# JunweiLiang/Multiverse

Measured on AMD Instinct MI355X. Metric: trajectories/sec (8-obs/12-pred, multi-scale 18x32+9x16 grid, greedy forward), higher is better.
Workload: dtype f16x3 (fp32 operands as two pre-scaled fp16 planes, fp32 accumulate and state; winograd F(3,3) over image rows on pre-transformed operands, 1.67 fp16 MFMAs issued per fp32 product over the gate kernels; error vs fp64 within 2x of the fp32-MFMA path's -- asserted under checkpoint-like dynamic range (; 1 GPU; BASELINE configs[1]: multi-scale 18x32+9x16 (scene 36x64x11), batch 64/GPU, fp32 forward-only, beam 1, obs 8 / pred 12; gate convolution on the fp16 matrix pipe (f16x3 split, fp32-class error); batch_per_gpu=64, global_batch=64, obs_len=8, pred_len=12, parallelism=batch-sharded x1, no data-path collective

## Files before the change

### multiverse_amd/csrc/engine.hip

```cpp
#include "../../include/multiverse_hip.h"

#include <hip/hip_runtime.h>

#include <cmath>
#include <cstdio>
#include <cstdlib>
#include <cstring>
#include <algorithm>
#include <map>
#include <memory>
#include <mutex>
#include <set>
#include <string>
#include <tuple>
#include <vector>

#include "convlstm_mfma.h"
#include "convlstm_wgrad.h"
#include "convlstm_f16x3.h"
#include "convlstm_wino.h"
#include "convlstm_wino3.h"
#include "convlstm_generic.h"
#include "convlstm_wgrad_f16x3.h"
#include "kernels_misc.h"
#include "decode_tail.h"
#include "sparse_x.h"
#include "multifuture_decode.h"
#include "train_kernels.h"
#include "comm.h"

#include "engine_state.h"
#include "gate_plan.h"
#include "engine_setup.h"
#include "engine_forward.h"
#include "engine_io.h"


#include "engine_train.h"

namespace {

struct OpCtx {
  int device;
  hipStream_t stream = nullptr;
  explicit OpCtx(int dev) : device(dev) {
    HIP_CHECK(hipSetDevice(dev));
    HIP_CHECK(hipStreamCreate(&stream));
  }
  ~OpCtx() { if (stream) (void)hipStreamDestroy(stream); }
  template <typename T>
  void up(DevBuf<T>& b, const T* src, size_t n) {
    b.alloc(n ? n : 1);
    if (n) HIP_CHECK(hipMemcpy(b.p, src, n * sizeof(T), hipMemcpyHostToDevice));
  }
  template <typename T>
  void down(T* dst, const DevBuf<T>& b, size_t n) {
    HIP_CHECK(hipStreamSynchronize(stream));
    if (n) HIP_CHECK(hipMemcpy(dst, b.p, n * sizeof(T), hipMemcpyDeviceToHost));
  }
};

}


extern "C" {

int mv_abi_version(void) { return MV_ABI_VERSION; }

const char* mv_last_error(mv_handle h) {
  return h ? h->err.c_str() : g_create_error.c_str();
}

int mv_create(const mv_config* cfg, int device, mv_handle* out) {
  if (!cfg || !out) { g_create_error = "mv_create: NULL argument"; return 1; }
  *out = nullptr;
  mv_engine* e = nullptr;
  int rc = guarded(nullptr, [&] {
    validate_config(*cfg);
    int ndev = 0;
    HIP_CHECK(hipGetDeviceCount(&ndev));
    MV_REQUIRE(device >= 0 && device < ndev, "device %d not in [0,%d)", device, ndev);
    HIP_CHECK(hipSetDevice(device));
    hipDeviceProp_t prop;
    HIP_CHECK(hipGetDeviceProperties(&prop, device));
    MV_REQUIRE(strncmp(prop.gcnArchName, "gfx950", 6) == 0,
               "device %d is %s; this library contains gfx950 (MI355X) code only",
               device, prop.gcnArchName);
    e = new mv_engine();
    e->cfg = *cfg;
    e->device = device;
    HIP_CHECK(hipStreamCreate(&e->stream));
    build_param_table(e);
    alloc_buffers(e);
    if (cfg->beam_size > 1) {
      size_t K = 0;
      for (int s = 0; s < cfg->num_scales; ++s)
        if (e->sc[s].use) K = e->sc[s].K;
      ensure_beam_step_lds(device, ((size_t)2 * cfg->beam_size * K + 512) * sizeof(float));
    }
  });
  if (rc != 0) { delete e; return rc; }
  *out = e;
  return 0;
}

int mv_destroy(mv_handle h) {
  if (!h) return 0;
  (void)hipSetDevice(h->device);
  if (h->stream) (void)hipStreamSynchronize(h->stream);
  if (h->copy_stream) (void)hipStreamSynchronize(h->copy_stream);
  if (h->fetch_stream) (void)hipStreamSynchronize(h->fetch_stream);
  pipeline_destroy(h);
  h->drop_graphs();
  if (h->comm) {
    if (h->comm->stream) (void)hipStreamSynchronize(h->comm->stream);
    if (h->comm->comm) (void)mv::rccl().CommDestroy(h->comm->comm);
    if (h->comm->ready) (void)hipEventDestroy(h->comm->ready);
    if (h->comm->done) (void)hipEventDestroy(h->comm->done);
    if (h->comm->stream) (void)hipStreamDestroy(h->comm->stream);
    delete h->comm;
  }
  delete h->train;
  if (h->stream) (void)hipStreamDestroy(h->stream);
  delete h;
  return 0;
}

int mv_num_params(mv_handle h) { return h ? (int)h->params.size() : -1; }

int mv_param_info(mv_handle h, int32_t i, char* name_out, int32_t name_cap,
                  int64_t* shape_out) {
  if (!h || i < 0 || i >= (int)h->params.size()) return -1;
  Param* p = h->params[i].get();
  if (name_out && name_cap > 0) {
    strncpy(name_out, p->name.c_str(), name_cap - 1);
    name_out[name_cap - 1] = 0;
  }
  if (shape_out)
    for (size_t d = 0; d < 4; ++d) shape_out[d] = d < p->shape.size() ? p->shape[d] : 0;
  return (int)p->shape.size();
}

int mv_set_param(mv_handle h, const char* tf_name, const float* data,
                 const int64_t* shape, int32_t rank) {
  if (!h) return 1;
  return guarded(h, [&] {
    MV_REQUIRE(tf_name && data && shape, "mv_set_param: NULL argument");
    auto it = h->by_name.find(tf_name);
    MV_REQUIRE(it != h->by_name.end(), "unknown parameter '%s'", tf_name);
    Param* p = it->second;
    MV_REQUIRE(rank == (int)p->shape.size(), "parameter %s: rank %d, expected %zu",
               tf_name, rank, p->shape.size());
    for (int d = 0; d < rank; ++d)
      MV_REQUIRE(shape[d] == p->shape[d], "parameter %s: dim %d is %lld, expected %lld",
                 tf_name, d, (long long)shape[d], (long long)p->shape[d]);
    const size_t n = p->elems();
    p->host.assign(data, data + n);
    p->dev.alloc(n);
    HIP_CHECK(hipMemcpy(p->dev.p, data, n * sizeof(float), hipMemcpyHostToDevice));
    p->set = true;
    h->drop_graphs();
    h->train_packs_valid = false;
    for (int s = 0; s < h->cfg.num_scales; ++s) h->sc[s].wq_valid = h->sc[s].sx_valid = false;
    for (int s = 0; s < h->cfg.num_scales; ++s) {
      ScaleState& S = h->sc[s];
      for (ConvCell* cc : {&S.enc_cls, &S.enc_reg, &S.dec_cls, &S.dec_reg})
        if (cc->kernel == p) {
          cc->wpack.release(); cc->wp16.release(); cc->wx32.release();
          cc->wpb.release(); cc->wpbt.release(); cc->wx32u.release(); cc->wpw.release(); cc->wpw3.release();
          cc->host_stale = false;
        }
    }
  });
}

int mv_get_param(mv_handle h, const char* tf_name, float* out, int64_t capacity) {
  if (!h) return 1;
  return guarded(h, [&] {
    MV_REQUIRE(tf_name && out, "mv_get_param: NULL argument");
    auto it = h->by_name.find(tf_name);
    MV_REQUIRE(it != h->by_name.end(), "unknown parameter '%s'", tf_name);
    Param* p = it->second;
    MV_REQUIRE(p->set, "parameter %s not set", tf_name);
    MV_REQUIRE((size_t)capacity >= p->elems(), "buffer too small for %s", tf_name);
    HIP_CHECK(hipMemcpy(out, p->dev.p, p->elems() * sizeof(float), hipMemcpyDeviceToHost));
  });
}

int mv_upload_inputs(mv_handle h, const mv_inputs* in) {
  if (!h) return 1;
  return guarded(h, [&] {
    MV_REQUIRE(in, "mv_upload_inputs: NULL inputs");
    upload_inputs(h, in);
  });
}

int mv_set_grid_centers(mv_handle h, int32_t scale, const double* centers) {
  if (!h) return 1;
  return guarded(h, [&] {
    MV_REQUIRE(scale >= 0 && scale < h->cfg.num_scales && h->sc[scale].use,
               "mv_set_grid_centers: scale %d is not an enabled scale", scale);
    MV_REQUIRE(centers, "mv_set_grid_centers: NULL centers");
    ScaleState& S = h->sc[scale];
    S.centers.alloc((size_t)S.K * 2);
    HIP_CHECK(hipMemcpy(S.centers.p, centers, (size_t)S.K * 2 * sizeof(double),
                        hipMemcpyHostToDevice));
  });
}

int mv_upload_inputs_compact(mv_handle h, const mv_inputs_compact* in) {
  if (!h) return 1;
  return guarded(h, [&] {
    MV_REQUIRE(in, "mv_upload_inputs_compact: NULL inputs");
    upload_inputs_compact(h, in);
  });
}

int mv_run_greedy_resident(mv_handle h) {
  if (!h) return 1;
  return guarded(h, [&] {
    MV_REQUIRE(h->cfg.beam_size == 1, "engine was created for beam search");
    run_forward(h, false);
  });
}

int mv_run_beam_resident(mv_handle h) {
  if (!h) return 1;
  return guarded(h, [&] { run_forward(h, true); });
}

int mv_synchronize(mv_handle h) {
  if (!h) return 1;
  return guarded(h, [&] {
    HIP_CHECK(hipStreamSynchronize(h->stream));
    drain_events(h);
  });
}

int mv_download_outputs(mv_handle h, mv_outputs* out) {
  if (!h) return 1;
  return guarded(h, [&] {
    MV_REQUIRE(out, "NULL outputs");
    download_outputs(h, out);
  });
}

int mv_download_beam_outputs(mv_handle h, mv_beam_outputs* out) {
  if (!h) return 1;
  return guarded(h, [&] {
    MV_REQUIRE(out, "NULL outputs");
    download_beam(h, out);
  });
}

int mv_decode_trajectories(mv_handle h, int32_t scale, int32_t center_only, double* out) {
  if (!h) return 1;
  return guarded(h, [&] {
    decode_trajectories(h, scale, center_only != 0, out);
    drain_events(h);
  });
}

int mv_beam_occupancy(mv_handle h, float* out) {
  if (!h) return 1;
  return guarded(h, [&] {
    beam_occupancy(h, out);
    drain_events(h);
  });
}

int mv_download_beam_ids(mv_handle h, int32_t* ids, float* logprobs) {
  if (!h) return 1;
  return guarded(h, [&] {
    download_beam_ids(h, ids, logprobs);
    drain_events(h);
  });
}

int mv_forward_greedy(mv_handle h, const mv_inputs* in, mv_outputs* out) {
  if (!h) return 1;
  return guarded(h, [&] {
    MV_REQUIRE(in && out, "mv_forward_greedy: NULL argument");
    MV_REQUIRE(h->cfg.beam_size == 1, "engine was created for beam search");
    upload_inputs(h, in);
    run_forward(h, false);
    download_outputs(h, out);
    drain_events(h);
  });
}

int mv_pipeline_create(mv_handle h, int32_t depth) {
  if (!h) return 1;
  return guarded(h, [&] { pipeline_create(h, depth); });
}

int mv_submit_greedy(mv_handle h, const mv_inputs* in) {
  if (!h) return 1;
  return guarded(h, [&] {
    MV_REQUIRE(in, "mv_submit_greedy: NULL argument");
    pipeline_submit(h, in);
  });
}

int mv_collect_greedy(mv_handle h, mv_outputs* out, int32_t* pred_len) {
  if (!h) return 1;
  return guarded(h, [&] {
    MV_REQUIRE(out, "mv_collect_greedy: NULL argument");
    if (pred_len && !h->pipe.empty())
      *pred_len = h->pipe[h->pipe_tail % h->pipe.size()].pred_len;
    pipeline_collect(h, out);
    drain_events(h);
  });
}

int mv_forward_beam(mv_handle h, const mv_inputs* in, mv_beam_outputs* out) {
  if (!h) return 1;
  return guarded(h, [&] {
    MV_REQUIRE(in && out, "mv_forward_beam: NULL argument");
    upload_inputs(h, in);
    run_forward(h, true);
    download_beam(h, out);
    drain_events(h);
  });
}

int mv_set_profiling(mv_handle h, int32_t enabled) {
  if (!h) return 1;
  h->profiling = enabled != 0;
  return 0;
}

int mv_train_init(mv_handle h, const mv_train_config* tc) {
  if (!h) return 1;
  return guarded(h, [&] {
    MV_REQUIRE(tc, "mv_train_init: NULL config");
    MV_REQUIRE(tc->optimizer >= 0 && tc->optimizer <= 3, "Optimizer not implemented: %d "
               "(0 adadelta, 1 momentum, 2 adam, 3 rmsprop; reference pred_models.py:1667-1681)",
               tc->optimizer);
    MV_REQUIRE(tc->class_feedback >= 0 && tc->class_feedback <= 2, "class_feedback %d",
               tc->class_feedback);
    MV_REQUIRE(tc->keep_prob > 0.f && tc->keep_prob <= 1.f, "keep_prob %g not in (0, 1]",
               tc->keep_prob);
    if (tc->use_soft_grid_class)
      MV_REQUIRE(tc->soft_kernel_size == 3 || tc->soft_kernel_size == 5,
                 "soft_kernel_size %d (3 or 5)", tc->soft_kernel_size);
    MV_REQUIRE(h->cfg.beam_size == 1, "training needs a greedy (beam_size 1) engine "
               "(reference pred_models.py:261)");
    if (!h->train) {
      h->train = new mv_train_holder();
      train_alloc(h);
      h->drop_graphs();
      for (int s = 0; s < h->cfg.num_scales; ++s) h->sc[s].wq_valid = h->sc[s].sx_valid = false;
    }
    TrainState& t = h->train->st;
    t.tc = *tc;
    if (t.slots_for != tc->optimizer) {
      HIP_CHECK(hipMemsetAsync(t.accum.p, 0, t.total_elems * sizeof(float), h->stream));
      HIP_CHECK(hipMemsetAsync(t.accum_update.p, 0, t.total_elems * sizeof(float), h->stream));
      if (tc->optimizer == 3)
        hipLaunchKernelGGL(mv::fill_kernel, dim3(cdiv(t.total_elems, 256)), dim3(256), 0,
                           h->stream, t.accum.p, 1.0f, t.total_elems);
      t.beta1_power = 0.9f; t.beta2_power = 0.999f;
      HIP_CHECK(hipStreamSynchronize(h->stream));
      t.slots_for = tc->optimizer;
    }
  });
}

int mv_train_forward_backward(mv_handle h, const mv_inputs* in, const mv_targets* tg,
                              mv_losses* out) {
  if (!h) return 1;
  return guarded(h, [&] {
    MV_REQUIRE((in == nullptr) == (tg == nullptr),
               "mv_train_forward_backward: give both inputs and targets, or neither "
               "(resident)");
    train_fwd_bwd(h, in, tg, out);
  });
}

int mv_upload_targets(mv_handle h, const mv_targets* tg) {
  if (!h) return 1;
  return guarded(h, [&] {
    MV_REQUIRE(h->train, "mv_train_init has not been called");
    MV_REQUIRE(tg, "mv_upload_targets: NULL targets");
    MV_REQUIRE(h->inputs_ready, "mv_upload_inputs first (it fixes T_pred)");
    upload_targets(h, tg);
    TS(h).targets_ready = true;
  });
}

int mv_upload_targets_compact(mv_handle h, const mv_targets_compact* tg) {
  if (!h) return 1;
  return guarded(h, [&] {
    MV_REQUIRE(h->train, "mv_train_init has not been called");
    MV_REQUIRE(tg, "mv_upload_targets_compact: NULL targets");
    MV_REQUIRE(h->inputs_ready, "mv_upload_inputs first (it fixes T_pred)");
    upload_targets_compact(h, tg);
    TS(h).targets_ready = true;
  });
}

int mv_train_apply(mv_handle h, float grad_scale) {
  if (!h) return 1;
  return guarded(h, [&] { train_apply(h, grad_scale); });
}

int mv_train_step(mv_handle h, const mv_inputs* in, const mv_targets* tg, mv_losses* out) {
  if (!h) return 1;
  return guarded(h, [&] {
    MV_REQUIRE((in == nullptr) == (tg == nullptr),
               "mv_train_step: give both inputs and targets, or neither (resident)");
    train_fwd_bwd(h, in, tg, out);
    train_apply(h, h->comm ? 1.0f / (float)h->comm->world : 1.0f);
  });
}

int mv_grad_buffer(mv_handle h, float** device_ptr, int64_t* elems) {
  if (!h) return 1;
  return guarded(h, [&] {
    MV_REQUIRE(h->train, "mv_train_init has not been called");
    MV_REQUIRE(device_ptr && elems, "mv_grad_buffer: NULL argument");
    *device_ptr = TS(h).grad.p;
    *elems = (int64_t)TS(h).total_elems;
  });
}

static Param* find_param(mv_handle h, const char* tf_name) {
  MV_REQUIRE(tf_name, "NULL parameter name");
  auto it = h->by_name.find(tf_name);
  MV_REQUIRE(it != h->by_name.end(), "unknown parameter '%s'", tf_name);
  return it->second;
}

int mv_get_grad(mv_handle h, const char* tf_name, float* out, int64_t capacity) {
  if (!h) return 1;
  return guarded(h, [&] {
    MV_REQUIRE(h->train && TS(h).have_grads, "no gradients (mv_train_forward_backward)");
    Param* p = find_param(h, tf_name);
    MV_REQUIRE(out && (size_t)capacity >= p->elems(), "buffer too small for %s", tf_name);
    HIP_CHECK(hipMemcpy(out, grad_of(h, p), p->elems() * sizeof(float),
                        hipMemcpyDeviceToHost));
  });
}

int mv_get_global_step(mv_handle h, int64_t* step) {
  if (!h || !step || !h->train) return 1;
  *step = h->train->st.global_step;
  return 0;
}

int mv_set_global_step(mv_handle h, int64_t step) {
  if (!h || !h->train) return 1;
  h->train->st.global_step = step;
  return 0;
}

int mv_comm_unique_id(uint8_t* id_out) {
  return guarded(nullptr, [&] {
    MV_REQUIRE(id_out, "mv_comm_unique_id: NULL buffer");
    mv::RcclApi& r = mv::rccl();
    MV_REQUIRE(r.ok, "RCCL unavailable: %s", r.error.c_str());
    ncclUniqueId id;
    ncclResult_t rc = r.GetUniqueId(&id);
    MV_REQUIRE(rc == ncclSuccess, "ncclGetUniqueId: %s", r.GetErrorString(rc));
    static_assert(sizeof(id) == MV_COMM_ID_BYTES, "ncclUniqueId size");
    memcpy(id_out, &id, sizeof(id));
  });
}

int mv_allreduce_init(mv_handle h, int32_t rank, int32_t world, const uint8_t* unique_id) {
  if (!h) return 1;
  return guarded(h, [&] {
    MV_REQUIRE(unique_id && world >= 1 && rank >= 0 && rank < world,
               "mv_allreduce_init: bad arguments (rank %d of %d)", rank, world);
    MV_REQUIRE(!h->comm, "mv_allreduce_init: communicator already initialised");
    mv::RcclApi& r = mv::rccl();
    MV_REQUIRE(r.ok, "RCCL unavailable: %s", r.error.c_str());
    std::unique_ptr<mv::Comm> c(new mv::Comm());
    c->rank = rank; c->world = world;
    ncclUniqueId id;
    memcpy(&id, unique_id, sizeof(id));
    ncclResult_t rc = r.CommInitRank(&c->comm, world, id, rank);
    MV_REQUIRE(rc == ncclSuccess, "ncclCommInitRank(rank %d of %d): %s", rank, world,
               r.GetErrorString(rc));
    HIP_CHECK(hipStreamCreateWithFlags(&c->stream, hipStreamNonBlocking));
    HIP_CHECK(hipEventCreateWithFlags(&c->ready, hipEventDisableTiming));
    HIP_CHECK(hipEventCreateWithFlags(&c->done, hipEventDisableTiming));
    h->comm = c.release();
  });
}

int mv_allreduce_info(mv_handle h, int32_t* rank, int32_t* world, int32_t* buckets,
                      double* bytes) {
  if (!h || !h->comm) return 1;
  if (rank) *rank = h->comm->rank;
  if (world) *world = h->comm->world;
  if (buckets) *buckets = h->comm->buckets_last;
  if (bytes) *bytes = h->comm->bytes_last;
  return 0;
}

int mv_attack_begin(mv_handle h) {
  if (!h) return 1;
  return guarded(h, [&] {
    MV_REQUIRE(!h->no_scene(), "mv_attack_begin: the model has no scene encoder (scene_conv_dim 0): "
               "there are no scene features");
    MV_REQUIRE(h->train, "mv_train_init has not been called");
    MV_REQUIRE(h->inputs_ready, "no inputs uploaded");
    TrainState& t = TS(h);
    const size_t n = (size_t)h->num_frames * h->cfg.scene_h * h->cfg.scene_w * h->cfg.scene_class;
    t.scene_clean.alloc((size_t)h->cfg.batch_size * h->cfg.obs_len * h->cfg.scene_h *
                        h->cfg.scene_w * h->cfg.scene_class);
    HIP_CHECK(hipMemcpyAsync(t.scene_clean.p, h->scene_feat.p, n * sizeof(float),
                             hipMemcpyDeviceToDevice, h->stream));
    t.want_dscene = true;
    t.have_dscene = false;
  });
}

int mv_attack_end(mv_handle h) {
  if (!h || !h->train) return 1;
  TS(h).want_dscene = false;
  return 0;
}

int mv_set_scene_feat(mv_handle h, const float* scene_feat) {
  if (!h) return 1;
  return guarded(h, [&] {
    MV_REQUIRE(!h->no_scene(), "mv_set_scene_feat: the model has no scene encoder (scene_conv_dim 0): "
               "there are no scene features");
    MV_REQUIRE(scene_feat && h->inputs_ready, "mv_set_scene_feat: NULL / no inputs uploaded");
    const size_t n = (size_t)h->num_frames * h->cfg.scene_h * h->cfg.scene_w * h->cfg.scene_class;
    HIP_CHECK(hipMemcpy(h->scene_feat.p, scene_feat, n * sizeof(float), hipMemcpyHostToDevice));
  });
}

int mv_get_scene_feat(mv_handle h, float* out) {
  if (!h) return 1;
  return guarded(h, [&] {
    MV_REQUIRE(!h->no_scene(), "mv_get_scene_feat: the model has no scene encoder (scene_conv_dim 0): "
               "there are no scene features");
    MV_REQUIRE(out && h->inputs_ready, "mv_get_scene_feat: NULL / no inputs uploaded");
    const size_t n = (size_t)h->num_frames * h->cfg.scene_h * h->cfg.scene_w * h->cfg.scene_class;
    HIP_CHECK(hipStreamSynchronize(h->stream));
    HIP_CHECK(hipMemcpy(out, h->scene_feat.p, n * sizeof(float), hipMemcpyDeviceToHost));
  });
}

int mv_get_scene_grad(mv_handle h, float* out) {
  if (!h) return 1;
  return guarded(h, [&] {
    MV_REQUIRE(!h->no_scene(), "mv_get_scene_grad: the model has no scene encoder (scene_conv_dim 0): "
               "there are no scene features");
    MV_REQUIRE(h->train && TS(h).have_dscene, "no input gradient (mv_attack_begin, then "
               "mv_train_forward_backward)");
    const size_t n = (size_t)h->num_frames * h->cfg.scene_h * h->cfg.scene_w * h->cfg.scene_class;
    HIP_CHECK(hipStreamSynchronize(h->stream));
    HIP_CHECK(hipMemcpy(out, TS(h).dscene.p, n * sizeof(float), hipMemcpyDeviceToHost));
  });
}

int mv_attack_step(mv_handle h, float epsilon, float step) {
  if (!h) return 1;
  return guarded(h, [&] {
    MV_REQUIRE(!h->no_scene(), "mv_attack_step: the model has no scene encoder (scene_conv_dim 0): "
               "there are no scene features");
    MV_REQUIRE(h->train && TS(h).have_dscene && TS(h).scene_clean.p,
               "mv_attack_step: mv_attack_begin + mv_train_forward_backward first");
    const size_t n = (size_t)h->num_frames * h->cfg.scene_h * h->cfg.scene_w * h->cfg.scene_class;
    hipLaunchKernelGGL(mv::adv_step_kernel, dim3(cdiv(n, 256)), dim3(256), 0, h->stream,
                       h->scene_feat.p, TS(h).dscene.p, TS(h).scene_clean.p, epsilon, step, n);
    HIP_CHECK(hipGetLastError());
  });
}

int mv_scene_mix(mv_handle h, const float* other, float weight) {
  if (!h) return 1;
  return guarded(h, [&] {
    MV_REQUIRE(!h->no_scene(), "mv_scene_mix: the model has no scene encoder (scene_conv_dim 0): "
               "there are no scene features");
    MV_REQUIRE(h->train && h->inputs_ready, "mv_scene_mix: training engine with inputs");
    const size_t n = (size_t)h->num_frames * h->cfg.scene_h * h->cfg.scene_w * h->cfg.scene_class;
    TrainState& t = TS(h);
    const float* src = t.scene_clean.p;
    DevBuf<float> tmp;
    if (other) {
      tmp.alloc(n);
      HIP_CHECK(hipMemcpy(tmp.p, other, n * sizeof(float), hipMemcpyHostToDevice));
      src = tmp.p;
    }
    MV_REQUIRE(src, "mv_scene_mix: no clean copy (mv_attack_begin)");
    hipLaunchKernelGGL(mv::mix_kernel, dim3(cdiv(n, 256)), dim3(256), 0, h->stream,
                       h->scene_feat.p, src, weight, n);
    HIP_CHECK(hipStreamSynchronize(h->stream));
  });
}

int mv_get_sample_losses(mv_handle h, int32_t scale, float* out) {
  if (!h) return 1;
  return guarded(h, [&] {
    MV_REQUIRE(h->train && TS(h).have_grads, "no losses (mv_train_forward_backward)");
    MV_REQUIRE(scale >= 0 && scale < h->cfg.num_scales && h->sc[scale].use && out,
               "mv_get_sample_losses: scale %d", scale);
    const int N = h->cfg.batch_size, Tp = h->pred_len;
    TrainState& t = TS(h);
    hipLaunchKernelGGL(mv::loss_rows_mean_kernel, dim3(cdiv(N, 256)), dim3(256), 0, h->stream,
                       t.sc[scale].loss_row.p, t.scratch.p, Tp, N);
    HIP_CHECK(hipStreamSynchronize(h->stream));
    HIP_CHECK(hipMemcpy(out, t.scratch.p, N * sizeof(float), hipMemcpyDeviceToHost));
  });
}

int mv_set_label_mixup(mv_handle h, const int32_t* const* obs_labels2,
                       const int32_t* const* pred_labels2, float weight,
                       const float* sample_weight) {
  if (!h) return 1;
  return guarded(h, [&] {
    MV_REQUIRE(!h->no_scene(), "mv_set_label_mixup: not built for a model without the scene encoder "
               "(scene_conv_dim 0)");
    MV_REQUIRE(h->train, "mv_train_init has not been called");
    MV_REQUIRE(obs_labels2 && pred_labels2, "mv_set_label_mixup: NULL argument");
    MV_REQUIRE(weight >= 0.f && weight <= 1.f, "mv_set_label_mixup: weight %g not in [0, 1]",
               (double)weight);
    TrainState& t = TS(h);
    const int N = h->cfg.batch_size, To = h->cfg.obs_len, Tp = h->pred_len;
    for (int s = 0; s < h->cfg.num_scales; ++s) {
      if (!h->sc[s].use) continue;
      MV_REQUIRE(obs_labels2[s] && pred_labels2[s], "mv_set_label_mixup: scale %d is NULL", s);
      const int K = h->sc[s].K;
      for (int i = 0; i < N * To; ++i)
        MV_REQUIRE(obs_labels2[s][i] >= 0 && obs_labels2[s][i] < K,
                   "mv_set_label_mixup: observed label %d out of range", obs_labels2[s][i]);
      for (int i = 0; i < N * Tp; ++i)
        MV_REQUIRE(pred_labels2[s][i] >= 0 && pred_labels2[s][i] < K,
                   "mv_set_label_mixup: future label %d out of range", pred_labels2[s][i]);
      HIP_CHECK(hipMemcpy(t.sc[s].obs_labels2.p, obs_labels2[s], (size_t)N * To * sizeof(int32_t),
                          hipMemcpyHostToDevice));
      HIP_CHECK(hipMemcpy(t.sc[s].pred_labels2.p, pred_labels2[s],
                          (size_t)N * Tp * sizeof(int32_t), hipMemcpyHostToDevice));
    }
    if (sample_weight)
      HIP_CHECK(hipMemcpy(t.sample_w.p, sample_weight, (size_t)N * sizeof(float),
                          hipMemcpyHostToDevice));
    t.mix_on = true; t.mix_sw = sample_weight != nullptr; t.mix_w = weight;
  });
}

int mv_clear_label_mixup(mv_handle h) {
  if (!h || !h->train) return 1;
  TS(h).mix_on = TS(h).mix_sw = false;
  TS(h).mix_w = 1.f;
  return 0;
}

int mv_set_dropout_seed(mv_handle h, uint32_t seed) {
  if (!h || !h->train) return 1;
  h->train->st.dropout_seed = seed;
  return 0;
}

int mv_get_opt_scalars(mv_handle h, float* beta1_power, float* beta2_power) {
  if (!h || !h->train || !beta1_power || !beta2_power) return 1;
  *beta1_power = h->train->st.beta1_power;
  *beta2_power = h->train->st.beta2_power;
  return 0;
}

int mv_set_opt_scalars(mv_handle h, float beta1_power, float beta2_power) {
  if (!h || !h->train) return 1;
  h->train->st.beta1_power = beta1_power;
  h->train->st.beta2_power = beta2_power;
  return 0;
}

int mv_get_opt_slot(mv_handle h, const char* tf_name, int32_t slot, float* out,
                    int64_t capacity) {
  if (!h) return 1;
  return guarded(h, [&] {
    MV_REQUIRE(h->train, "mv_train_init has not been called");
    MV_REQUIRE(slot == 0 || slot == 1, "slot must be 0 or 1 (see multiverse_hip.h)");
    Param* p = find_param(h, tf_name);
    MV_REQUIRE(out && (size_t)capacity >= p->elems(), "buffer too small for %s", tf_name);
    const float* src = (slot == 0 ? TS(h).accum.p : TS(h).accum_update.p) +
                       TS(h).goff[param_index(h, p)];
    HIP_CHECK(hipMemcpy(out, src, p->elems() * sizeof(float), hipMemcpyDeviceToHost));
  });
}

int mv_set_opt_slot(mv_handle h, const char* tf_name, int32_t slot, const float* data,
                    int64_t elems) {
  if (!h) return 1;
  return guarded(h, [&] {
    MV_REQUIRE(h->train, "mv_train_init has not been called");
    MV_REQUIRE(slot == 0 || slot == 1, "slot must be 0 or 1 (see multiverse_hip.h)");
    Param* p = find_param(h, tf_name);
    MV_REQUIRE(data && (size_t)elems == p->elems(), "size mismatch for %s", tf_name);
    float* dst = (slot == 0 ? TS(h).accum.p : TS(h).accum_update.p) +
                 TS(h).goff[param_index(h, p)];
    HIP_CHECK(hipMemcpy(dst, data, p->elems() * sizeof(float), hipMemcpyHostToDevice));
  });
}

int mv_set_compute_mode(mv_handle h, int32_t mode) {
  if (!h) return 1;
  return guarded(h, [&] {
    MV_REQUIRE(mode >= 0 && mode <= 2, "compute mode %d (0 = fp32 MFMA, 1 = f16x3, 2 = bf16)",
               mode);
    MV_REQUIRE(mode == 0 || h->cfg.convlstm_kernel == 3,
               "compute mode %d needs convlstm_kernel 3 (%d given: the matrix-pipe gate kernels "
               "are 3 x 3 stencils; mode 0 runs the generic fp32 loops)", mode,
               h->cfg.convlstm_kernel);
    if (mode != 0) {
      const mv_config& c = h->cfg;
      size_t K = 0;
      for (int s = 0; s < c.num_scales; ++s)
        if (h->sc[s].use) K = std::max(K, (size_t)h->sc[s].K);
      const size_t xc = (size_t)std::max(c.scene_conv_dim, c.emb_size);
      for (int i = 0; i < mv::kMaxGroup; ++i) {
        const size_t rows = (size_t)c.batch_size * ((i % 2 == 0) ? c.beam_size : 1);
        h->px16[i].alloc(2 * (rows * K * xc + mv::kPlaneSlack + mv::kPlanePad));
        h->ph16[i].alloc(2 * (rows * K * c.hidden_size + mv::kPlaneSlack + mv::kPlanePad));
        HIP_CHECK(hipMemset(h->px16[i].p, 0, h->px16[i].n * sizeof(_Float16)));
        if (c.activation != 0) h->xexp[i].alloc(65);
        if (wino3_possible(mode, c.activation)) {
          size_t vx = 0, vh = 0;
          for (int s = 0; s < c.num_scales; ++s) {
            if (!h->sc[s].use) continue;
            vx = std::max(vx, wino3_scratch_elems((int)rows, h->sc[s].H, h->sc[s].W, (int)xc));
            vh = std::max(vh, wino3_scratch_elems((int)rows, h->sc[s].H, h->sc[s].W, c.hidden_size));
          }
          if (vx) h->pv3x[i].alloc(vx);
          if (vh) h->pv3h[i].alloc(vh);
        }
        HIP_CHECK(hipMemset(h->ph16[i].p, 0, h->ph16[i].n * sizeof(_Float16)));
      }
    }
    if (mode != 0 && h->planes.empty()) {
      for (int s = 0; s < h->cfg.num_scales; ++s) {
        ScaleState& S = h->sc[s];
        if (!S.use) continue;
        for (DevBuf<float>* b : {&S.cls_h[0], &S.cls_h[1], &S.reg_h[0], &S.reg_h[1],
                                 &S.cls_hg, &S.xbuf_cls, &S.xbuf_reg}) {
          if (!b->p) continue;
          h->plane_store.emplace_back(new DevBuf<_Float16>());
          DevBuf<_Float16>& pb = *h->plane_store.back();
          pb.alloc(2 * (b->n + mv::kPlaneSlack + mv::kPlanePad));
          HIP_CHECK(hipMemset(pb.p, 0, pb.n * sizeof(_Float16)));
          h->planes[b->p] = mv_engine::PlaneBuf{pb.p + mv::kPlanePad,
                                                b->n + mv::kPlaneSlack + mv::kPlanePad, false};
          if (b == &S.xbuf_cls || b == &S.xbuf_reg) h->xbufs.insert(b->p);
        }
      }
    }
    for (auto& kv : h->planes) kv.second.valid = false;
    if (h->compute_mode != mode) {
      h->drop_graphs();
      h->train_packs_valid = false;
    }
    h->compute_mode = mode;
  });
}

int mv_set_graph_mode(mv_handle h, int32_t enabled) {
  if (!h) return 1;
  h->graph_mode = enabled != 0;
  return 0;
}

int mv_reset_kernel_stats(mv_handle h) {
  if (!h) return 1;
  return guarded(h, [&] {
    HIP_CHECK(hipStreamSynchronize(h->stream));
    drain_events(h);
    h->stats.clear();
  });
}

int mv_num_kernel_stats(mv_handle h) { return h ? (int)h->stats.size() : -1; }

int mv_kernel_stat_dense_flops(mv_handle h, int32_t i, double* flops_dense) {
  if (!h || i < 0 || i >= (int)h->stats.size() || !flops_dense) return 1;
  *flops_dense = h->stats[i].flops_dense;
  return 0;
}

int mv_kernel_stat_mfma_flops(mv_handle h, int32_t i, double* flops_mfma) {
  if (!h || i < 0 || i >= (int)h->stats.size() || !flops_mfma) return 1;
  *flops_mfma = h->stats[i].flops_mfma;
  return 0;
}

int mv_kernel_stat(mv_handle h, int32_t i, char* name_out, int32_t name_cap,
                   int64_t* launches, double* total_ms, double* flops, double* bytes) {
  if (!h || i < 0 || i >= (int)h->stats.size()) return 1;
  const KernelStat& s = h->stats[i];
  if (name_out && name_cap > 0) {
    strncpy(name_out, s.name.c_str(), name_cap - 1);
    name_out[name_cap - 1] = 0;
  }
  if (launches) *launches = s.launches;
  if (total_ms) *total_ms = s.total_ms;
  if (flops) *flops = s.flops;
  if (bytes) *bytes = s.bytes;
  return 0;
}

static int time_resident(mv_handle h, int32_t iters, float* ms_out, bool beam) {
  if (!h) return 1;
  return guarded(h, [&] {
    MV_REQUIRE(iters >= 1 && ms_out, "bad arguments");
    hipEvent_t a, b;
    HIP_CHECK(hipEventCreate(&a));
    HIP_CHECK(hipEventCreate(&b));
    HIP_CHECK(hipEventRecord(a, h->stream));
    for (int i = 0; i < iters; ++i) run_forward(h, beam);
    HIP_CHECK(hipEventRecord(b, h->stream));
    HIP_CHECK(hipEventSynchronize(b));
    HIP_CHECK(hipEventElapsedTime(ms_out, a, b));
    (void)hipEventDestroy(a);
    (void)hipEventDestroy(b);
    drain_events(h);
  });
}

int mv_time_greedy_resident(mv_handle h, int32_t iters, float* ms_out) {
  return time_resident(h, iters, ms_out, false);
}
int mv_time_beam_resident(mv_handle h, int32_t iters, float* ms_out) {
  return time_resident(h, iters, ms_out, true);
}

}

#include "engine_ops.h"
```

### multiverse_amd/csrc/engine_forward.h

```cpp
#pragma once

namespace {


using mv::ConvLstmArgs;

void set_sparse_x(mv_engine* e, ScaleState& S, ConvLstmArgs& a, bool decoder,
                  const int32_t* hot, int hot_stride, int hot_div) {
  a.sx_bias = decoder ? S.sx_dec_bias.p : nullptr;
  a.sx_corr = decoder ? S.sx_dec_corr.p : S.sx_enc_corr.p;
  a.sx_hot = hot; a.sx_hot_stride = hot_stride; a.sx_hot_div = hot_div;
  a.sx_cellyx = S.sx_cellyx.p;
  a.sx_rad = decoder ? 2 : 1;
  a.sx_by_class = decoder ? 1 : 0;
}

ConvLstmArgs conv_problem(mv_engine* e, const ConvCell& cc, const float* x,
                          const float* h, const float* c, const int32_t* src_row_h,
                          const int32_t* src_row_c, float* h_out, float* c_out,
                          int rows, int H, int W, bool zero_state,
                          size_t x_row_stride = 0, bool want_h16 = true) {
  ConvLstmArgs a{};
  const size_t xrs = x_row_stride ? x_row_stride : (size_t)H * W * cc.Cx;
  MV_REQUIRE((size_t)rows * H * W * e->cfg.hidden_size < ((size_t)1 << 31) &&
             (size_t)rows * xrs < ((size_t)1 << 31),
             "ConvLSTM state of %d rows exceeds the 2^31-element addressing of one "
             "launch; lower batch_size x beam_size", rows);
  a.x_row_stride = (int32_t)xrs;
  a.x = x; a.h = h; a.c = c; a.src_row_h = src_row_h; a.src_row_c = src_row_c;
  a.wpack = cc.wpack.p; a.bias = cc.biases->dev.p;
  a.h_out = h_out; a.c_out = c_out;
  a.rows = rows; a.H = H; a.W = W; a.Cx = cc.Cx; a.C = e->cfg.hidden_size;
  mv::convlstm_finish_args(a, zero_state);
  a.want_h16 = want_h16 ? 1 : 0;
  return a;
}

ConvCell* cell_of_bias(mv_engine* e, const float* bias) {
  for (int s = 0; s < e->cfg.num_scales; ++s) {
    ScaleState& S = e->sc[s];
    if (!S.use) continue;
    for (ConvCell* cc : active_cells(e, S))
      if (cc->biases && cc->biases->dev.p == bias) return cc;
  }
  throw HipError{"internal: unknown ConvLSTM cell"};
}

ConvCell* cell_of_pack(mv_engine* e, const float* wpack) {
  for (int s = 0; s < e->cfg.num_scales; ++s) {
    ScaleState& S = e->sc[s];
    for (ConvCell* cc : active_cells(e, S))
      if (cc->wpack.p == wpack) return cc;
  }
  throw HipError{"internal: unknown weight pack"};
}


void prepare_gate_operands(mv_engine* e, const std::vector<ConvLstmArgs>& probs,
                           const std::vector<ConvCell*>& cells,
                           std::vector<mv::ConvLstm16Args>& p16) {
  struct SplitItem { const float* in; _Float16* p0; _Float16* p1; int cells, C; };
  std::vector<SplitItem> splits;
  struct DynItem { const float* in; _Float16* p0; _Float16* p1; int cells, C; int32_t* bits; };
  std::vector<DynItem> dyn_splits;
  const bool bf16 = e->compute_mode == 2;
  auto ready = [&](const float* src) -> const mv_engine::PlaneBuf* {
    auto it = e->planes.find(src);
    return (it != e->planes.end() && it->second.valid) ? &it->second : nullptr;
  };
  for (size_t i = 0; i < probs.size(); ++i) {
    const ConvLstmArgs& a = probs[i];
    mv::ConvLstm16Args& q = p16[i];
    MV_REQUIRE(a.H * a.W >= 32, "f16x3 / bf16 compute modes need grids of at least 32 cells "
               "(%d x %d); use compute mode f32", a.H, a.W);
    MV_REQUIRE((double)a.rows * a.H * a.W * a.C * 4.0 < 4294967296.0,
               "f16x3 / bf16 compute modes: state tensor of %d rows exceeds 4 GB", a.rows);
    MV_REQUIRE(!a.gates_out || (double)a.rows * a.H * a.W * a.C * 16.0 < 4294967296.0,
               "f16x3 / bf16 training forward: gate tensor of %d rows exceeds 4 GB "
               "(lower the per-GPU batch or use compute mode f32)", a.rows);
    q.f = a;
    q.wp16 = bf16 ? cells[i]->wpb.p : cells[i]->wp16.p;
    q.wx32 = bf16 ? cells[i]->wx32u.p : cells[i]->wx32.p;
    const size_t ncell = (size_t)a.rows * a.H * a.W;
    const int xpass = bf16_x_passes(e->compute_mode, e->dyn_x(), a.x_small);
    q.n_xk = a.x_small ? 0 : xpass * mv::f16x3_xksteps(a.Cx);
    q.n_hk = a.zero_state ? 0 : 9 * (a.C / 16);
    q.w_ksteps = (a.x_small ? 0 : xpass * mv::f16x3_xksteps(a.Cx)) + 9 * (a.C / 16);
    if (bf16)
      MV_REQUIRE((q.n_xk / 3) % MV_BF16_UNITS == 0 && (q.n_hk / 3) % MV_BF16_UNITS == 0,
                 "bf16 mode: %d x / %d h k-steps do not fill whole LDS stages (emb_size and "
                 "scene_conv_dim must be multiples of 32)", q.n_xk, q.n_hk);
    q.x16 = nullptr; q.h16 = nullptr;
    q.x_plane_stride = q.h_plane_stride = 0;
    q.h16_out = nullptr;
    q.h16_out_stride = 0;
    e->plane_invalidate(a.h_out);
    if (gate_knobs().epi_planes && a.want_h16 && !a.gates_out) {
      size_t pst = 0;
      if (_Float16* po = e->plane_out(a.h_out, &pst)) {
        q.h16_out = po;
        q.h16_out_stride = (int64_t)pst;
      }
    }
    q.f.skip_h32 = (a.skip_h32 && q.h16_out && !e->train) ? 1 : 0;
    if (has_dense_x(a)) {
      MV_REQUIRE((size_t)a.x_row_stride == (size_t)a.H * a.W * a.Cx,
                 "internal: f16x3 needs a contiguous x operand");
      if (const auto* pb = ready(a.x)) {
        q.x16 = pb->p; q.x_plane_stride = (int64_t)pb->n;
      } else {
        const size_t pst = ncell * a.Cx + mv::kPlaneSlack + mv::kPlanePad;
        MV_REQUIRE(e->px16[i].n >= 2 * pst, "internal: f16x3 x plane scratch");
        _Float16* p0 = e->px16[i].p + mv::kPlanePad;
        q.x16 = p0; q.x_plane_stride = (int64_t)pst;
        if (e->dyn_x()) {
          MV_REQUIRE(e->xexp[i].p, "internal: x exponent scratch");
          q.x_exp = e->xexp[i].p + 64;
          dyn_splits.push_back(DynItem{a.x, p0, p0 + pst, (int)ncell, a.Cx, e->xexp[i].p});
        } else {
          splits.push_back(SplitItem{a.x, p0, bf16 ? (_Float16*)nullptr : p0 + pst, (int)ncell, a.Cx});
        }
      }
      MV_REQUIRE(!(bf16 && e->dyn_x()) || q.x_exp, "internal: bf16 mode, unbounded activations: "
                 "a dense x operand came as producer planes, without its exponent");
    }
    if (!a.zero_state) {
      if (const auto* pb = ready(a.h)) {
        q.h16 = pb->p; q.h_plane_stride = (int64_t)pb->n;
      } else {
        const size_t pst = ncell * a.C + mv::kPlaneSlack + mv::kPlanePad;
        MV_REQUIRE(e->ph16[i].n >= 2 * pst, "internal: f16x3 h plane scratch");
        _Float16* p0 = e->ph16[i].p + mv::kPlanePad;
        q.h16 = p0; q.h_plane_stride = (int64_t)pst;
        splits.push_back(SplitItem{a.h, p0, bf16 ? (_Float16*)nullptr : p0 + pst, (int)ncell, a.C});
      }
    }
  }
  for (const DynItem& it : dyn_splits) {
    launch(e, "split_planes", 0, 12.0 * (double)it.cells * it.C, [&] {
      HIP_CHECK(hipMemsetAsync(it.bits, 0, 64 * sizeof(int32_t), e->stream));
      hipLaunchKernelGGL(mv::absmax_bits_kernel, dim3(256), dim3(256), 0, e->stream, it.in,
                         (size_t)it.cells * it.C, it.bits);
      hipLaunchKernelGGL(mv::split_planes_dyn_kernel,
                         dim3(mv::split_planes_blocks((size_t)it.cells, it.C)), dim3(256), 0,
                         e->stream, it.in, it.p0, it.p1, it.cells, it.C, it.bits, it.bits + 64);
    });
  }
  for (size_t s0 = 0; s0 < splits.size(); s0 += mv::kSplitGroup) {
    mv::SplitGroup g{};
    double sbytes = 0;
    unsigned nb = 0;
    g.n = (int)std::min<size_t>(mv::kSplitGroup, splits.size() - s0);
    for (int j = 0; j < g.n; ++j) {
      const SplitItem& it = splits[s0 + j];
      g.in[j] = it.in; g.p0[j] = it.p0; g.p1[j] = it.p1; g.M[j] = it.cells; g.C[j] = it.C;
      nb += mv::split_planes_blocks((size_t)it.cells, it.C);
      g.blk_end[j] = nb;
      sbytes += (bf16 ? 6.0 : 8.0) * (double)it.cells * it.C;
    }
    launch(e, "split_planes", 0, sbytes, [&] {
      hipLaunchKernelGGL(mv::split_planes_group_kernel, dim3(nb), dim3(256), 0, e->stream, g);
    });
  }
}

double queue_wino3_transform(std::vector<mv::Wn3TransformItem>& tr, const mv::Wn3TransformItem& it) {
  tr.push_back(it);
  return (double)it.rows * it.H * it.W * it.Cc * 4.0 * (1.0 + 5.0 / 3.0);
}

void launch_gate_group(const ForwardPlan& pl, const mv::ConvLstm16Args* p16,
                       const _Float16* const* packs, const float* const* w_hwio,
                       _Float16* const* v3x, _Float16* const* v3h, int n, hipStream_t stream) {
  if (pl.form == GateForm::Direct16)
    return mv::launch_convlstm16_steps(p16, n, pl.shift, pl.map_mode, stream);
  if (pl.form == GateForm::Bf16)
    return mv::launch_convlstm_bf16_steps(p16, n, pl.shift, pl.map_mode, pl.x_passes == 3, stream);
  mv::ConvLstmWinoArgs pw[mv::kMaxGroup] = {};
  for (int i = 0; i < n; ++i) {
    pw[i].b = p16[i];
    pw[i].wpw = packs[i];
    pw[i].w_hwio = w_hwio[i];
    pw[i].n_xc = p16[i].f.x_small ? 0 : p16[i].f.Cx / 16;
    pw[i].v3x = v3x ? v3x[i] : nullptr;
    pw[i].v3h = v3h ? v3h[i] : nullptr;
  }
  if (pl.form == GateForm::Wino2) mv::launch_convlstm_wino_steps(pw, n, pl.map_mode, stream);
  else if (pl.form == GateForm::Wino3)
    mv::launch_convlstm_wino3_steps(pw, n, pl.halo, pl.map_mode, stream);
  else mv::launch_convlstm_bf16t_steps(pw, n, pl.halo, pl.map_mode, stream);
}

void run_conv_group_f16x3(mv_engine* e, const std::vector<ConvLstmArgs>& probs,
                          double flops, double bytes, double dense) {
  const int n = (int)probs.size();
  MV_REQUIRE(n <= mv::kMaxGroup, "internal: gate group of %d problems", n);
  std::vector<ConvCell*> cells(n);
  for (int i = 0; i < n; ++i) cells[i] = cell_of_pack(e, probs[i].wpack);
  std::vector<mv::ConvLstm16Args> p16(n);
  prepare_gate_operands(e, probs, cells, p16);
  ForwardProblem fp[mv::kMaxGroup];
  for (int i = 0; i < n; ++i) fp[i] = ForwardProblem{&p16[i], cells[i], e->pv3x[i].n, e->pv3h[i].n};
  const ForwardPlan pl = plan_forward_group(e->compute_mode, fp, n);
  const _Float16* packs[mv::kMaxGroup] = {};
  const float* w_hwio[mv::kMaxGroup] = {};
  _Float16 *v3x[mv::kMaxGroup] = {}, *v3h[mv::kMaxGroup] = {};
  std::vector<mv::Wn3TransformItem> tr3;
  double tr3_bytes = 0;
  for (int i = 0; i < n; ++i) {
    const mv::ConvLstm16Args& q = p16[i];
    const ConvLstmArgs& a = q.f;
    w_hwio[i] = cells[i]->kernel->dev.p;
    packs[i] = pl.form == GateForm::Wino2 ? cells[i]->wpw.p
             : pl.form == GateForm::Wino3 ? cells[i]->wpw3.p
             : pl.form == GateForm::Bf16T ? cells[i]->wpbt.p : nullptr;
    if (pl.form != GateForm::Wino3) continue;
    if (!a.zero_state) {
      v3h[i] = e->pv3h[i].p;
      tr3_bytes += queue_wino3_transform(tr3, {q.h16, q.h_plane_stride, v3h[i], a.src_row_h,
                                               a.rows, a.H, a.W, a.C});
    }
    if (has_dense_x(a)) {
      v3x[i] = e->pv3x[i].p;
      tr3_bytes += queue_wino3_transform(tr3, {q.x16, q.x_plane_stride, v3x[i], nullptr,
                                               a.rows, a.H, a.W, a.Cx});
    }
  }
  if (!tr3.empty())
    launch(e, "wino3_transform", 0, tr3_bytes, [&] {
      mv::launch_wino3_transforms(tr3.data(), (int)tr3.size(), e->stream);
    });
  launch(e, "convlstm_step", flops, bytes, [&] {
    launch_gate_group(pl, p16.data(), packs, w_hwio, v3x, v3h, n, e->stream);
  }, dense, pl.mfma_factor);
}

void run_conv_group(mv_engine* e, const std::vector<ConvLstmArgs>& probs) {
  if (probs.empty()) return;
  double flops = 0, bytes = 0, dense = 0;
  for (const auto& a : probs) {
    const double M = (double)a.rows * a.H * a.W;
    dense += 2.0 * M * 9.0 * (a.Cx + a.C) * 4.0 * a.C;
    const double cx = a.sx_corr ? 0.0 : (double)a.Cx;
    flops += 2.0 * M * 9.0 * (cx + (a.zero_state ? 0 : a.C)) * 4.0 * a.C;
    bytes += M * (cx + (a.zero_state ? 2.0 : 4.0) * a.C) * 4.0;
  }
  if (e->compute_mode != 0) {
    run_conv_group_f16x3(e, probs, flops, bytes, dense);
    return;
  }
  if (e->cfg.convlstm_kernel != 3) {
    const double kk = (double)e->cfg.convlstm_kernel * e->cfg.convlstm_kernel / 9.0;
    launch(e, "convlstm_step", flops * kk, bytes, [&] {
      for (const auto& a : probs) {
        mv::ConvGenericArgs ga{};
        ga.f = a;
        ga.w = cell_of_bias(e, a.bias)->kernel->dev.p;
        ga.ksize = e->cfg.convlstm_kernel;
        mv::launch_convlstm_generic_step(ga, e->stream);
      }
    }, dense * kk, 0.0);
    return;
  }
  launch(e, "convlstm_step", flops, bytes, [&] {
    mv::launch_convlstm_steps(probs.data(), (int)probs.size(), e->stream);
  }, dense, 1.0);
}

void run_scene(mv_engine* e) {
  const mv_config& c = e->cfg;
  const int U = e->num_frames;
  const float* in = e->scene_feat.p;
  int Hi = c.scene_h, Wi = c.scene_w, Ci = c.scene_class;
  const int k = c.scene_conv_kernel;
  for (int i = 0; i < c.num_scales; ++i) {
    const int Ho = e->conv_h[i], Wo = e->conv_w[i], Co = c.scene_conv_dim;
    const int pad_h = std::max((Ho - 1) * 2 + k - Hi, 0);
    const int pad_w = std::max((Wo - 1) * 2 + k - Wi, 0);
    const size_t total = (size_t)U * Ho * Wo * Co;
    float* out = e->scene_conv[i].p;
    const float *w = e->scene_W[i]->dev.p, *b = e->scene_b[i]->dev.p;
    if (k == 1 && Co <= 64) {
      const size_t M = (size_t)U * Ho * Wo;
      launch(e, "scene_proj1x1_mfma", 2.0 * M * Ci * Co,
             4.0 * (total + (double)M * Ci), [&] {
        hipLaunchKernelGGL(mv::scene_proj1x1_mfma_kernel, dim3(cdiv(M, 128)), dim3(256), 0,
                           e->stream, in, w, b, out, U, Hi, Wi, Ci, Ho, Wo, Co, c.activation);
      });
    } else {
    launch(e, "scene_conv_s2_tanh", 2.0 * total * k * k * Ci,
           4.0 * (total + (double)U * Hi * Wi * Ci), [&] {
      hipLaunchKernelGGL(mv::scene_conv_s2_tanh_kernel, dim3(cdiv(total, 256)),
                         dim3(256), 0, e->stream, in, w, b, out, U, Hi, Wi, Ci,
                         Ho, Wo, Co, k, pad_h / 2, pad_w / 2, c.activation);
    });
    }
    in = out; Hi = Ho; Wi = Wo; Ci = Co;
  }
  for (int s = 0; s < c.num_scales; ++s) {
    ScaleState& S = e->sc[s];
    if (!S.use) continue;
    const size_t total = (size_t)c.batch_size * S.K * c.scene_conv_dim;
    launch(e, "scene_mean", (double)total * c.obs_len,
           4.0 * total * (c.obs_len + 1), [&] {
      hipLaunchKernelGGL(mv::scene_mean_kernel, dim3(cdiv(total, 256)), dim3(256),
                         0, e->stream, e->scene_conv[s].p, e->obs_scene.p,
                         S.scene_mean.p, c.batch_size, c.obs_len, S.K,
                         c.scene_conv_dim);
    });
  }
}

struct Cursors {
  int cls[MV_MAX_SCALES] = {0, 0};
  int reg[MV_MAX_SCALES] = {0, 0};
};

static bool beam_shared_first() {
  static const bool on =
      !(getenv("MV_BEAM_SHARED_FIRST") && atoi(getenv("MV_BEAM_SHARED_FIRST")) == 0);
  return on;
}

void run_encoders(mv_engine* e, Cursors& cur) {
  const mv_config& c = e->cfg;
  const int N = c.batch_size, T = c.obs_len, D = c.scene_conv_dim;
  for (int t = 0; t < T; ++t) {
    std::vector<ConvLstmArgs> probs;
    for (int s = 0; s < c.num_scales; ++s) {
      ScaleState& S = e->sc[s];
      if (!S.use) continue;
      const size_t total = (size_t)N * S.K * D;
      const bool sparse = sparse_x_on(e, S);
      const size_t nc = (size_t)N * 9 * 4 * c.hidden_size;
      if (e->no_scene()) {
        if (!sparse) {
          const int E = S.enc_cls.Cx;
          const size_t tx = (size_t)N * S.K * E;
          launch(e, "enc_grid_emb_onehot", (double)tx, 4.0 * tx, [&] {
            size_t pst = 0;
            _Float16* p16 = e->plane_out(S.xbuf_cls.p, &pst);
            hipLaunchKernelGGL(mv::enc_grid_emb_onehot_kernel, dim3(cdiv(tx, 256)), dim3(256),
                               0, e->stream, S.labels.p, T, t, 1, e->enc_emb_W->dev.p,
                               e->enc_emb_b->dev.p, S.xbuf_cls.p, N, S.H, S.W, E, p16, pst,
                               c.activation);
          });
        }
      } else if (sparse) {
        if (t == 0)
          launch(e, "sx_encoder_corr", 2.0 * nc * D * T, 4.0 * nc * T, [&] {
            hipLaunchKernelGGL(mv::sx_encoder_corr_kernel,
                               dim3(cdiv((size_t)4 * c.hidden_size, 256), 9,
                                    cdiv((size_t)N, mv::kSxRows) * T),
                               dim3(256), 0, e->stream, S.enc_cls.kernel->dev.p,
                               e->scene_conv[s].p, e->obs_scene.p, S.labels.p, N, T, -1, S.K, D,
                               c.hidden_size, S.sx_enc_corr.p);
          });
      } else {
      launch(e, "enc_class_input", 0, 4.0 * total, [&] {
        size_t pst = 0;
        _Float16* p16 = e->plane_out(S.xbuf_cls.p, &pst);
        hipLaunchKernelGGL(mv::enc_class_input_kernel, dim3(cdiv(total, 256)),
                           dim3(256), 0, e->stream, e->scene_conv[s].p,
                           e->obs_scene.p, S.labels.p, S.xbuf_cls.p, N, T, t, S.K, D, p16,
                           pst);
      });
      }
      const size_t row = (size_t)S.K * 2;
      const int cc = cur.cls[s], cr = cur.reg[s];
      probs.push_back(conv_problem(e, S.enc_cls, S.xbuf_cls.p, S.cls_h[cc].p,
                                   S.cls_c[cc].p, nullptr, nullptr, S.cls_h[cc ^ 1].p,
                                   S.cls_c[cc ^ 1].p, N, S.H, S.W, t == 0, 0,
                                   t + 1 < T || !c.use_gnn));
      probs.back().skip_h32 =
          (t + 1 < T || (!c.use_gnn && (c.beam_size == 1 || beam_shared_first()))) ? 1 : 0;
      if (sparse && e->no_scene()) {
        set_sparse_x(e, S, probs.back(), true, S.labels.p + t, T, 1);
        probs.back().sx_bias = S.sx_enc_bias.p;
        probs.back().sx_corr = S.sx_enc_tab.p;
      } else if (sparse) {
        set_sparse_x(e, S, probs.back(), false, S.labels.p + t, T, 1);
        probs.back().sx_corr = S.sx_enc_corr.p + (size_t)t * nc;
      }
      if (!c.use_single_decoder)
        probs.push_back(conv_problem(e, S.enc_reg, S.obs_reg.p + (size_t)t * row,
                                     S.reg_h[cr].p, S.reg_c[cr].p, nullptr, nullptr,
                                     S.reg_h[cr ^ 1].p, S.reg_c[cr ^ 1].p, N, S.H, S.W,
                                     t == 0, (size_t)T * row));
      if (!c.use_single_decoder) probs.back().skip_h32 = 1;
      cur.cls[s] ^= 1; cur.reg[s] ^= 1;
    }
    run_conv_group(e, probs);
  }
}

static int gnn_version() {
  const char* v = getenv("MV_GNN");
  if (v && strcmp(v, "v1") == 0) return 1;
  if (v && strcmp(v, "v2") == 0) return 2;
  return 3;
}

struct GnnJob {
  ScaleState* S; const float* h; const int32_t* src_row; float* out; int rows, sm_div;
  const int32_t* row_ref = nullptr;
};

void run_gnn_jobs(mv_engine* e, const std::vector<GnnJob>& jobs) {
  const mv_config& c = e->cfg;
  static const int env_ver = gnn_version();
  const size_t max_rows = (size_t)c.batch_size * (size_t)std::max(1, c.beam_size);
  auto v3_ok = [&](const GnnJob& J) {
    return (gnn_scene_dim(e) == 0 || gnn_scene_dim(e) == 64) &&
           max_rows * J.S->K * c.hidden_size * 4 < ((size_t)1 << 32);
  };
  for (size_t j0 = 0; j0 < jobs.size();) {
    const GnnJob& A = jobs[j0];
    const bool tiled = env_ver >= 2 && A.S->W <= 32 && c.hidden_size == 256 && c.scene_conv_dim <= 64;
    size_t nj = 1;
    if (tiled && j0 + 1 < jobs.size() && jobs[j0 + 1].S->W <= 32) nj = 2;
    const int ver = env_ver >= 3 && !(v3_ok(A) && (nj == 1 || v3_ok(jobs[j0 + 1]))) ? 2 : env_ver;
    mv::GnnGroup grp{};
    double flops = 0, bytes = 0;
    unsigned nblocks = 0;
    for (size_t j = 0; j < nj; ++j) {
      const GnnJob& J = jobs[j0 + j];
      const size_t cells = (size_t)J.rows * J.S->K;
      size_t pst = 0;
      _Float16* p16 = e->plane_out(J.out, &pst);
      const bool need_f32 = !(tiled && p16 && !e->train && e->compute_mode != 0);
      flops += cells * (9.0 * 2 * 2 * (c.hidden_size + gnn_scene_dim(e)) +
                        9.0 * 2 * c.hidden_size);
      bytes += 4.0 * cells * c.hidden_size *
                   (1.0 + (need_f32 ? 1.0 : 0.0) + (p16 ? 1.0 : 0.0)) +
               4.0 * (cells / J.sm_div) * gnn_scene_dim(e);
      int ng = 0;
      const unsigned nb = ver >= 3 ? mv::gnn_v3_blocks(cells, &ng) : mv::gnn_v2_blocks(cells, &ng);
      mv::GnnProblem& P = grp.p[j];
      P.h = J.h; P.scene_mean = J.S->scene_mean.p; P.src_row = J.src_row;
      P.out = need_f32 ? J.out : nullptr; P.p16 = p16; P.p16_stride = pst;
      P.M = J.rows; P.H = J.S->H; P.W = J.S->W; P.sm_div = J.sm_div; P.ngroups = ng;
      P.row_ref = J.row_ref;
      if (j == 0) grp.nblocks0 = nb;
      nblocks += nb;
    }
    if (nj == 1) grp.nblocks0 = nblocks;
    launch(e, "gnn_attend", flops, bytes, [&] {
      if (tiled && ver >= 3) {
        hipLaunchKernelGGL(mv::gnn_attend_v3_kernel, dim3(nblocks), dim3(mv::kGnn3Threads), 0,
                           e->stream, grp, c.hidden_size, gnn_scene_dim(e));
      } else if (tiled) {
        hipLaunchKernelGGL(mv::gnn_attend_v2_kernel, dim3(nblocks), dim3(mv::kGnnThreads), 0, e->stream,
                           grp, c.hidden_size, gnn_scene_dim(e));
      } else {
        const size_t cells = (size_t)A.rows * A.S->K;
        size_t pst = 0;
        _Float16* p16 = e->plane_out(A.out, &pst);
        if (c.hidden_size <= 256)
          hipLaunchKernelGGL(mv::gnn_attend_kernel<1>, dim3(cdiv(cells, 4)), dim3(256), 0,
                             e->stream, A.h, A.S->scene_mean.p, A.src_row, A.out, A.rows,
                             A.S->H, A.S->W, c.hidden_size, gnn_scene_dim(e), A.sm_div, p16, pst);
        else
          hipLaunchKernelGGL(mv::gnn_attend_kernel<2>, dim3(cdiv(cells, 4)), dim3(256), 0,
                             e->stream, A.h, A.S->scene_mean.p, A.src_row, A.out, A.rows,
                             A.S->H, A.S->W, c.hidden_size, gnn_scene_dim(e), A.sm_div, p16, pst);
      }
    });
    j0 += nj;
  }
}

void run_gnn(mv_engine* e, ScaleState& S, const float* h, const int32_t* src_row,
             float* out, int rows, int sm_div) {
  run_gnn_jobs(e, {GnnJob{&S, h, src_row, out, rows, sm_div}});
}

template <int P>
void run_hidden2grid(mv_engine* e, ScaleState& S, const float* h, const float* w,
                     float* out, size_t out_row_stride, int rows) {
  const size_t cells = (size_t)rows * S.K;
  const int C = e->cfg.hidden_size;
  launch(e, "hidden2grid", cells * 2.0 * 9 * C * P, 4.0 * cells * (C + P), [&] {
    hipLaunchKernelGGL(mv::hidden2grid_kernel<P>, dim3(cdiv(cells, 4)), dim3(256),
                       0, e->stream, h, w, out, out_row_stride, rows, S.H, S.W, C);
  });
}

static bool tail_v2() {
  static const bool on = !(getenv("MV_TAIL") && strcmp(getenv("MV_TAIL"), "v1") == 0);
  return on;
}

void run_emb_onehot(mv_engine* e, ScaleState& S, const int32_t* ids, int stride,
                    float* out, int rows, int ids_div = 1) {
  const int E = e->cfg.emb_size;
  const size_t total = (size_t)rows * S.K * E;
  launch(e, "grid_emb_onehot", (double)total, 4.0 * total, [&] {
    size_t pst = 0;
    _Float16* p16 = e->plane_out(out, &pst);
    if (tail_v2() && E % 8 == 0)
      hipLaunchKernelGGL(mv::grid_emb_onehot8_kernel, dim3(cdiv(total / 8, 256)), dim3(256), 0,
                         e->stream, ids, stride, ids_div, S.emb_cls_W->dev.p,
                         S.emb_cls_b->dev.p, out, rows, S.H, S.W, E, p16, pst, e->cfg.activation);
    else
      hipLaunchKernelGGL(mv::grid_emb_onehot_kernel, dim3(cdiv(total, 256)),
                         dim3(256), 0, e->stream, ids, stride, ids_div, S.emb_cls_W->dev.p,
                         S.emb_cls_b->dev.p, out, rows, S.H, S.W, E, p16, pst, e->cfg.activation);
  });
}

void run_emb_dense(mv_engine* e, ScaleState& S, const float* x, size_t row_stride,
                   float* out, int rows, Param* W = nullptr, Param* b = nullptr, int P = 2) {
  const int E = e->cfg.emb_size;
  const size_t total = (size_t)rows * S.K * E;
  if (!W) { W = S.emb_reg_W; b = S.emb_reg_b; }
  launch(e, "grid_emb_dense", total * 2.0 * 9 * P, 4.0 * total, [&] {
    size_t pst = 0;
    _Float16* p16 = e->plane_out(out, &pst);
    hipLaunchKernelGGL(mv::grid_emb_dense_kernel, dim3(cdiv(total, 256)), dim3(256),
                       0, e->stream, x, row_stride, W->dev.p, b->dev.p, out, rows, S.H, S.W,
                       P, E, p16, pst, e->cfg.activation);
  });
}

ConvLstmArgs reg_decoder_problem(mv_engine* e, int s, Cursors& cur, int t, int Tp,
                                 bool embed = true) {
  const mv_config& c = e->cfg;
  ScaleState& S = e->sc[s];
  const int N = c.batch_size, T = c.obs_len;
  const size_t orow = (size_t)Tp * S.K * 2;
  if (t == 0)
    run_emb_dense(e, S, S.obs_reg.p + (size_t)(T - 1) * S.K * 2, (size_t)T * S.K * 2,
                  S.xbuf_reg.p, N);
  else if (embed)
    run_emb_dense(e, S, S.out_reg.p + (size_t)(t - 1) * S.K * 2, orow, S.xbuf_reg.p, N);
  const int cr = cur.reg[s];
  cur.reg[s] ^= 1;
  return conv_problem(e, S.dec_reg, S.xbuf_reg.p, S.reg_h[cr].p, S.reg_c[cr].p, nullptr,
                      nullptr, S.reg_h[cr ^ 1].p, S.reg_c[cr ^ 1].p, N, S.H, S.W, false);
}

void reg_decoder_output(mv_engine* e, int s, const Cursors& cur, int t, int Tp) {
  ScaleState& S = e->sc[s];
  const size_t orow = (size_t)Tp * S.K * 2;
  run_hidden2grid<2>(e, S, S.reg_h[cur.reg[s]].p, S.out_reg_W->dev.p,
                     S.out_reg.p + (size_t)t * S.K * 2, orow, e->cfg.batch_size);
}

struct TailPlan {
  int s;
  const float* cls_h; int cls_rows; float* cls_out; int64_t cls_stride;
  bool cls_next;
  const float* reg_h; float* reg_out; int64_t reg_stride; bool reg_next;
  int reg_rows = 0;
  int32_t* cls_ids_out = nullptr; float* cls_x_out = nullptr; float* reg_x_out = nullptr;
  bool cls_embed = true;
};

void run_tail(mv_engine* e, const std::vector<TailPlan>& plans) {
  const mv_config& c = e->cfg;
  const int C = c.hidden_size, E = c.emb_size, N = c.batch_size;
  std::vector<mv::H2gQProblem> qp;
  std::vector<mv::TailProblem> tp;
  double qbytes = 0, qflops = 0, tbytes = 0;
  for (const TailPlan& pl : plans) {
    ScaleState& S = e->sc[pl.s];
    MV_REQUIRE((size_t)S.K * 2 <= 2048 && E % 16 == 0 && E <= 512,
               "decode tail: K %d / emb_size %d", S.K, E);
    const int reg_rows = pl.reg_rows ? pl.reg_rows : N;
    const size_t cc = (size_t)pl.cls_rows * S.K, cr = (size_t)reg_rows * S.K;
    qp.push_back(mv::H2gQProblem{pl.cls_h, S.wq_cls.p, S.q_cls.p, (int32_t)cc, 1});
    qp.push_back(mv::H2gQProblem{pl.reg_h, S.wq_reg.p, S.q_reg.p, (int32_t)cr, 2});
    qbytes += 4.0 * (cc * (C + 9.0) + cr * (C + 18.0));
    qflops += 2.0 * 9 * C * (cc + 2.0 * cr);
    mv::TailProblem a{};
    a.q = S.q_cls.p; a.out = pl.cls_out; a.out_row_stride = pl.cls_stride;
    a.rows = pl.cls_rows; a.H = S.H; a.W = S.W; a.P = 1; a.E = E; a.onehot = 1;
    a.act = c.activation;
    tbytes += 4.0 * cc * (9 + 1);
    if (pl.cls_next) {
      a.ids_out = pl.cls_ids_out ? pl.cls_ids_out : S.ids.p;
      if (pl.cls_x_out) {
        if (pl.cls_embed) {
          a.emb_w = S.emb_cls_W->dev.p; a.emb_b = S.emb_cls_b->dev.p;
          a.x_out = pl.cls_x_out;
          tbytes += 4.0 * cc * E;
        }
      } else if (!sparse_x_on(e, S)) {
        size_t pst = 0;
        a.emb_w = S.emb_cls_W->dev.p; a.emb_b = S.emb_cls_b->dev.p;
        a.x_out = S.xbuf_cls.p;
        a.x16 = e->plane_out(S.xbuf_cls.p, &pst); a.x16_stride = (int64_t)pst;
        tbytes += 4.0 * cc * E * (a.x16 ? 2 : 1);
      }
    }
    tp.push_back(a);
    mv::TailProblem b{};
    b.q = S.q_reg.p; b.out = pl.reg_out; b.out_row_stride = pl.reg_stride;
    b.rows = reg_rows; b.H = S.H; b.W = S.W; b.P = 2; b.E = E; b.onehot = 0;
    b.act = c.activation;
    tbytes += 4.0 * cr * (18 + 2);
    if (pl.reg_next) {
      size_t pst = 0;
      b.emb_w = S.emb_reg_W->dev.p; b.emb_b = S.emb_reg_b->dev.p;
      if (pl.reg_x_out) {
        b.x_out = pl.reg_x_out;
        tbytes += 4.0 * cr * E;
      } else {
      b.x_out = S.xbuf_reg.p;
      b.x16 = e->plane_out(S.xbuf_reg.p, &pst); b.x16_stride = (int64_t)pst;
      tbytes += 4.0 * cr * E * (b.x16 ? 2 : 1);
      }
    }
    tp.push_back(b);
  }
  MV_REQUIRE(qp.size() <= (size_t)mv::kTailMax, "decode tail: too many chains");
  launch(e, "hidden2grid", qflops, qbytes, [&] {
    mv::launch_h2g_q(qp.data(), (int)qp.size(), C, e->stream);
  });
  launch(e, "decode_tail", 0, tbytes, [&] {
    mv::launch_decode_tail(tp.data(), (int)tp.size(), e->stream);
  });
}

void run_decoders_greedy(mv_engine* e, Cursors& cur, int Tp) {
  const mv_config& c = e->cfg;
  const int N = c.batch_size, T = c.obs_len;
  const bool v2 = tail_v2();
  for (int t = 0; t < Tp; ++t) {
    std::vector<ConvLstmArgs> probs;
    if (c.use_gnn) {
      std::vector<GnnJob> jobs;
      for (int s = 0; s < c.num_scales; ++s)
        if (e->sc[s].use)
          jobs.push_back(GnnJob{&e->sc[s], e->sc[s].cls_h[cur.cls[s]].p, nullptr,
                                e->sc[s].cls_hg.p, N, 1});
      run_gnn_jobs(e, jobs);
    }
    for (int s = 0; s < c.num_scales; ++s) {
      ScaleState& S = e->sc[s];
      if (!S.use) continue;
      const int cc = cur.cls[s];
      const float* hin = c.use_gnn ? S.cls_hg.p : S.cls_h[cc].p;
      const bool sparse = sparse_x_on(e, S) && (t == 0 || !c.class_feedback_dense);
      if (sparse)
        ;
      else if (t == 0)
        run_emb_onehot(e, S, S.labels.p + (T - 1), T, S.xbuf_cls.p, N);
      else if (c.class_feedback_dense)
        run_emb_dense(e, S, S.out_cls.p + (size_t)(t - 1) * S.K, (size_t)Tp * S.K,
                      S.xbuf_cls.p, N, S.emb_cls_W, S.emb_cls_b, 1);
      else if (!v2)
        run_emb_onehot(e, S, S.ids.p, 1, S.xbuf_cls.p, N);
      probs.push_back(conv_problem(e, S.dec_cls, S.xbuf_cls.p, hin, S.cls_c[cc].p,
                                   nullptr, nullptr, S.cls_h[cc ^ 1].p,
                                   S.cls_c[cc ^ 1].p, N, S.H, S.W, false, 0,
                                   !c.use_gnn));
      if (sparse) {
        if (t == 0) set_sparse_x(e, S, probs.back(), true, S.labels.p + (T - 1), T, 1);
        else set_sparse_x(e, S, probs.back(), true, S.ids.p, 1, 1);
      }
      cur.cls[s] ^= 1;
      if (!c.use_single_decoder) probs.push_back(reg_decoder_problem(e, s, cur, t, Tp, !v2));
    }
    std::stable_sort(probs.begin(), probs.end(), [](const ConvLstmArgs& a, const ConvLstmArgs& b) {
      return (a.sx_corr == nullptr) > (b.sx_corr == nullptr);
    });
    run_conv_group(e, probs);
    if (v2) {
      std::vector<TailPlan> plans;
      for (int s = 0; s < c.num_scales; ++s) {
        ScaleState& S = e->sc[s];
        if (!S.use) continue;
        TailPlan pl{};
        pl.s = s;
        pl.cls_h = S.cls_h[cur.cls[s]].p; pl.cls_rows = N;
        pl.cls_out = S.out_cls.p + (size_t)t * S.K; pl.cls_stride = (int64_t)Tp * S.K;
        pl.cls_next = t + 1 < Tp && !c.class_feedback_dense;
        pl.reg_h = S.reg_h[cur.reg[s]].p;
        pl.reg_out = S.out_reg.p + (size_t)t * S.K * 2; pl.reg_stride = (int64_t)Tp * S.K * 2;
        pl.reg_next = t + 1 < Tp;
        if (c.use_single_decoder) {
          pl.reg_h = pl.cls_h;
          pl.reg_next = false;
        }
        plans.push_back(pl);
      }
      run_tail(e, plans);
      continue;
    }
    for (int s = 0; s < c.num_scales; ++s) {
      ScaleState& S = e->sc[s];
      if (!S.use) continue;
      const size_t orow = (size_t)Tp * S.K;
      float* logits = S.out_cls.p + (size_t)t * S.K;
      run_hidden2grid<1>(e, S, S.cls_h[cur.cls[s]].p, S.out_cls_W->dev.p, logits, orow, N);
      if (t + 1 < Tp && !c.class_feedback_dense) {
        launch(e, "argmax_rows", 0, 4.0 * N * S.K, [&] {
          hipLaunchKernelGGL(mv::argmax_rows_kernel, dim3(N), dim3(64), 0, e->stream,
                             logits, orow, S.ids.p, N, S.K);
        });
      }
      if (c.use_single_decoder)
        run_hidden2grid<2>(e, S, S.cls_h[cur.cls[s]].p, S.out_reg_W->dev.p,
                           S.out_reg.p + (size_t)t * S.K * 2, (size_t)Tp * S.K * 2, N);
      else
        reg_decoder_output(e, s, cur, t, Tp);
    }
  }
}

__global__ void tile_rows_kernel(const float* __restrict__ in, float* __restrict__ out,
                                 size_t row_elems4, int B, size_t total4) {
  const size_t idx = (size_t)blockIdx.x * blockDim.x + threadIdx.x;
  if (idx >= total4) return;
  const size_t r = idx / row_elems4, off = idx - r * row_elems4;
  reinterpret_cast<mv::f32x4_t*>(out)[idx] =
      reinterpret_cast<const mv::f32x4_t*>(in)[(r / B) * row_elems4 + off];
}

__global__ void tile_beam0_kernel(float* __restrict__ logits, int K, int B, size_t total) {
  const size_t idx = (size_t)blockIdx.x * blockDim.x + threadIdx.x;
  if (idx >= total) return;
  const size_t r = idx / K;
  if (r % B) logits[idx] = logits[(r - r % B) * K + (idx - r * K)];
}

__global__ void beam_backtrace_kernel(const int32_t* __restrict__ step_ids,
                                      const int32_t* __restrict__ step_parents,
                                      int32_t* __restrict__ out_ids,
                                      int32_t* __restrict__ trace, int N, int B,
                                      int T) {
  const int idx = blockIdx.x * blockDim.x + threadIdx.x;
  if (idx >= N * B) return;
  const int n = idx / B, b = idx - n * B;
  int par = b;
  for (int t = T - 1; t >= 0; --t) {
    const size_t o = ((size_t)t * N + n) * B + par;
    out_ids[((size_t)n * B + b) * T + t] = step_ids[o];
    trace[((size_t)n * B + b) * T + t] = par;
    par = step_parents[o];
  }
}

__global__ void beam_gather_logits_kernel(const float* __restrict__ step_logits,
                                          const int32_t* __restrict__ trace,
                                          float* __restrict__ out, int N, int B,
                                          int T, int K) {
  const size_t idx = (size_t)blockIdx.x * blockDim.x + threadIdx.x;
  const size_t total = (size_t)N * B * T * K;
  if (idx >= total) return;
  const int k = idx % K;
  size_t r = idx / K;
  const int t = r % T; r /= T;
  const int b = r % B;
  const int n = r / B;
  const int par = trace[((size_t)n * B + b) * T + t];
  out[idx] = step_logits[(((size_t)t * N + n) * B + par) * K + k];
}

void run_decoders_beam(mv_engine* e, int s, Cursors& cur, int Tp) {
  const mv_config& c = e->cfg;
  ScaleState& S = e->sc[s];
  const int N = c.batch_size, T = c.obs_len, B = c.beam_size, K = S.K,
            C = c.hidden_size;
  const int R = N * B;
  const bool shared_first = beam_shared_first();
  if (!shared_first) {
    const int cc = cur.cls[s];
    const size_t row4 = (size_t)K * C / 4, total4 = (size_t)R * row4;
    launch(e, "beam_tile_state", 0, 8.0 * total4 * 16, [&] {
      hipLaunchKernelGGL(tile_rows_kernel, dim3(cdiv(total4, 256)), dim3(256), 0,
                         e->stream, S.cls_h[cc].p, S.cls_h[cc ^ 1].p, row4, B, total4);
      hipLaunchKernelGGL(tile_rows_kernel, dim3(cdiv(total4, 256)), dim3(256), 0,
                         e->stream, S.cls_c[cc].p, S.cls_c[cc ^ 1].p, row4, B, total4);
    });
    e->plane_invalidate(S.cls_h[cc ^ 1].p);
    cur.cls[s] ^= 1;
  }
  HIP_CHECK(hipMemsetAsync(e->bm_lp[0].p, 0, (size_t)R * sizeof(float), e->stream));
  int lpi = 0;
  const int32_t* src = nullptr;
  const bool sparse = sparse_x_on(e, S);
  static const bool dedupe_env =
      !(getenv("MV_BEAM_GNN_DEDUPE") && atoi(getenv("MV_BEAM_GNN_DEDUPE")) == 0);
  const bool dedupe = dedupe_env && shared_first && c.use_gnn && K <= 64 * mv::kBeamRankJ &&
                      !(getenv("MV_BEAM_STEP") && strcmp(getenv("MV_BEAM_STEP"), "v1") == 0) &&
                      !(getenv("MV_GNN") && strcmp(getenv("MV_GNN"), "v1") == 0);
  for (int time = 0; time <= Tp; ++time) {
    const bool one_per_sample = shared_first && time <= 1;
    const int rows_now = one_per_sample ? N : R;
    if (time > 0) {
      const int cc = cur.cls[s];
      const float* hin = c.use_gnn ? S.cls_hg.p : S.cls_h[cc].p;
      std::vector<ConvLstmArgs> probs;
      probs.push_back(conv_problem(e, S.dec_cls, S.xbuf_cls.p, hin, S.cls_c[cc].p,
                                   (c.use_gnn && !dedupe) ? nullptr : src, src,
                                   S.cls_h[cc ^ 1].p, S.cls_c[cc ^ 1].p, rows_now, S.H, S.W,
                                   false, 0, !c.use_gnn));
      if (sparse) {
        if (time == 1)
          set_sparse_x(e, S, probs.back(), true, S.labels.p + (T - 1), T, one_per_sample ? 1 : B);
        else
          set_sparse_x(e, S, probs.back(), true, e->bm_ids.p + (size_t)(time - 2) * R, 1, 1);
      }
      cur.cls[s] ^= 1;
      const bool v2 = tail_v2();
      const bool single = c.use_single_decoder != 0;
      MV_REQUIRE(!single || v2, "use_single_decoder with beam search needs the v2 decoder tail");
      if (!single) probs.push_back(reg_decoder_problem(e, s, cur, time - 1, Tp, !v2));
      run_conv_group(e, probs);
      float* logits = e->bm_logits.p + (size_t)(time - 1) * R * K;
      float* regstep = single ? e->bm_reg_steps.p + (size_t)(time - 1) * R * K * 2 : nullptr;
      const size_t lrow = one_per_sample ? (size_t)B * K : (size_t)K;
      if (v2) {
        TailPlan pl{};
        pl.s = s;
        pl.cls_h = S.cls_h[cur.cls[s]].p; pl.cls_rows = rows_now;
        pl.cls_out = logits; pl.cls_stride = lrow; pl.cls_next = false;
        if (single) {
          pl.reg_h = pl.cls_h; pl.reg_rows = rows_now;
          pl.reg_out = regstep; pl.reg_stride = (int64_t)lrow * 2; pl.reg_next = false;
        } else {
        pl.reg_h = S.reg_h[cur.reg[s]].p;
        pl.reg_out = S.out_reg.p + (size_t)(time - 1) * K * 2;
        pl.reg_stride = (int64_t)Tp * K * 2; pl.reg_next = time < Tp;
        }
        run_tail(e, {pl});
      } else {
        reg_decoder_output(e, s, cur, time - 1, Tp);
        run_hidden2grid<1>(e, S, S.cls_h[cur.cls[s]].p, S.out_cls_W->dev.p, logits,
                           lrow, rows_now);
      }
      if (one_per_sample) {
        const size_t total = (size_t)R * K;
        hipLaunchKernelGGL(tile_beam0_kernel, dim3(cdiv(total, 256)), dim3(256), 0,
                           e->stream, logits, K, B, total);
        if (single)
          hipLaunchKernelGGL(tile_beam0_kernel, dim3(cdiv(total * 2, 256)), dim3(256), 0,
                             e->stream, regstep, K * 2, B, total * 2);
      }
      int32_t* ids = e->bm_ids.p + (size_t)(time - 1) * R;
      int32_t* parents = e->bm_parents.p + (size_t)(time - 1) * R;
      if (dedupe)
        HIP_CHECK(hipMemsetAsync(e->bm_ref.p, 0, (size_t)R * sizeof(int32_t), e->stream));
      launch(e, "beam_step", 0, 4.0 * R * K, [&] {
        launch_beam_step(e->stream, logits, e->bm_lp[lpi].p, e->bm_cand.p, N, B, K, time,
                         c.diverse_beam, logf(c.diverse_gamma), c.fix_num_timestep,
                         e->bm_lp[lpi ^ 1].p, ids, parents, e->bm_src_row.p,
                         one_per_sample ? 1 : B, dedupe ? e->bm_ref.p : nullptr);
      });
      lpi ^= 1;
      src = e->bm_src_row.p;
      if (time == Tp) break;
      if (!sparse) run_emb_onehot(e, S, ids, 1, S.xbuf_cls.p, R);
    } else if (sparse) {
    } else if (shared_first) {
      run_emb_onehot(e, S, S.labels.p + (T - 1), T, S.xbuf_cls.p, N, 1);
    } else {
      run_emb_onehot(e, S, S.labels.p + (T - 1), T, S.xbuf_cls.p, R, B);
    }
    if (c.use_gnn) {
      if (dedupe) {
        GnnJob job{&S, S.cls_h[cur.cls[s]].p, nullptr, S.cls_hg.p, rows_now,
                   one_per_sample ? 1 : B};
        job.row_ref = time >= 2 ? e->bm_ref.p : nullptr;
        run_gnn_jobs(e, {job});
      } else {
      const int out_rows = (shared_first && time == 0) ? N : R;
      run_gnn(e, S, S.cls_h[cur.cls[s]].p, src, S.cls_hg.p, out_rows,
              (shared_first && time == 0) ? 1 : B);
      }
    }
  }
  hipLaunchKernelGGL(beam_backtrace_kernel, dim3(cdiv(R, 256)), dim3(256), 0,
                     e->stream, e->bm_ids.p, e->bm_parents.p, e->bm_out_ids.p,
                     e->bm_trace.p, N, B, Tp);
  const size_t total = (size_t)R * Tp * K;
  hipLaunchKernelGGL(beam_gather_logits_kernel, dim3(cdiv(total, 256)), dim3(256), 0,
                     e->stream, e->bm_logits.p, e->bm_trace.p, e->bm_out_logits.p,
                     N, B, Tp, K);
  if (c.use_single_decoder) {
    const size_t tot2 = (size_t)R * Tp * K * 2;
    hipLaunchKernelGGL(beam_gather_logits_kernel, dim3(cdiv(tot2, 256)), dim3(256), 0,
                       e->stream, e->bm_reg_steps.p, e->bm_trace.p, e->bm_out_reg.p,
                       N, B, Tp, K * 2);
  }
  if (lpi != 0)
    HIP_CHECK(hipMemcpyAsync(e->bm_lp[0].p, e->bm_lp[1].p, (size_t)R * sizeof(float),
                             hipMemcpyDeviceToDevice, e->stream));
}

void enqueue_forward(mv_engine* e, bool beam) {
  const mv_config& c = e->cfg;
  const int Tp = e->pred_len;
  if (!e->no_scene()) run_scene(e);
  Cursors cur;
  run_encoders(e, cur);
  if (beam) {
    int s = 0;
    for (int i = 0; i < c.num_scales; ++i) if (e->sc[i].use) s = i;
    run_decoders_beam(e, s, cur, Tp);
  } else {
    run_decoders_greedy(e, cur, Tp);
  }
  HIP_CHECK(hipGetLastError());
}

void run_forward(mv_engine* e, bool beam) {
  MV_REQUIRE(e->inputs_ready, "no inputs uploaded (mv_upload_inputs)");
  ensure_params(e);
  if (beam)
    MV_REQUIRE(e->cfg.beam_size > 1, "engine was created with beam_size 1");
  if (!e->graph_mode || e->profiling) {
    enqueue_forward(e, beam);
    e->last_forward = beam ? 2 : 1;
    return;
  }
  const auto key = std::make_tuple(beam ? 1 : 0, e->pred_len, e->num_frames);
  auto it = e->graphs.find(key);
  if (it == e->graphs.end()) {
    hipGraph_t g = nullptr;
    HIP_CHECK(hipStreamBeginCapture(e->stream, hipStreamCaptureModeThreadLocal));
    try {
      enqueue_forward(e, beam);
    } catch (...) {
      (void)hipStreamEndCapture(e->stream, &g);
      if (g) (void)hipGraphDestroy(g);
      throw;
    }
    HIP_CHECK(hipStreamEndCapture(e->stream, &g));
    hipGraphExec_t ex = nullptr;
    hipError_t ie = hipGraphInstantiate(&ex, g, nullptr, nullptr, 0);
    (void)hipGraphDestroy(g);
    HIP_CHECK(ie);
    it = e->graphs.emplace(key, ex).first;
  }
  HIP_CHECK(hipGraphLaunch(it->second, e->stream));
  e->last_forward = beam ? 2 : 1;
}

}
```

### multiverse_amd/csrc/engine_setup.h

```cpp
#pragma once

namespace {

inline unsigned cdiv(size_t a, size_t b) { return (unsigned)((a + b - 1) / b); }

void ensure_beam_step_lds(int device, size_t lds) {
  static std::mutex mu;
  static std::map<int, size_t> granted;
  std::lock_guard<std::mutex> lk(mu);
  MV_REQUIRE(lds <= 160 * 1024, "beam_size*K too large for the LDS beam step (%zu B)", lds);
  size_t& cur = granted[device];
  if (lds > cur) {
    HIP_CHECK(hipFuncSetAttribute(reinterpret_cast<const void*>(mv::beam_step_kernel),
                                  hipFuncAttributeMaxDynamicSharedMemorySize, (int)lds));
    HIP_CHECK(hipFuncSetAttribute(reinterpret_cast<const void*>(mv::beam_select_kernel),
                                  hipFuncAttributeMaxDynamicSharedMemorySize, (int)lds));
    cur = lds;
  }
}

void launch_beam_step(hipStream_t stream, const float* logits, const float* prev_lp,
                      float* cand, int N, int B, int K, int time, int diverse,
                      float log_gamma, int fix_num_timestep, float* new_lp, int32_t* ids,
                      int32_t* parents, int32_t* src_row, int rows_per_sample,
                      int32_t* row_ref = nullptr) {
  static const bool v1 = getenv("MV_BEAM_STEP") && strcmp(getenv("MV_BEAM_STEP"), "v1") == 0;
  if (v1 || K > 64 * mv::kBeamRankJ || !cand) {
    hipLaunchKernelGGL(mv::beam_step_kernel, dim3(N), dim3(512),
                       ((size_t)2 * B * K + 512) * sizeof(float), stream, logits, prev_lp, B,
                       K, time, diverse, log_gamma, fix_num_timestep, new_lp, ids, parents,
                       src_row, rows_per_sample, row_ref);
    HIP_CHECK(hipGetLastError());
    return;
  }
  const int R = N * B;
  const dim3 grid(cdiv((size_t)R, 4)), block(256);
  if (K <= 64 * 3)
    hipLaunchKernelGGL(mv::beam_rank_kernel<3>, grid, block, 0, stream, logits, prev_lp, R, B,
                       K, time, diverse, log_gamma, cand);
  else if (K <= 64 * 9)
    hipLaunchKernelGGL(mv::beam_rank_kernel<9>, grid, block, 0, stream, logits, prev_lp, R, B,
                       K, time, diverse, log_gamma, cand);
  else
    hipLaunchKernelGGL(mv::beam_rank_kernel<mv::kBeamRankJ>, grid, block, 0, stream, logits,
                       prev_lp, R, B, K, time, diverse, log_gamma, cand);
  hipLaunchKernelGGL(mv::beam_select_kernel, dim3(N), dim3(1024),
                     ((size_t)B * K + 64) * sizeof(float), stream, cand, B, K, time,
                     fix_num_timestep, new_lp, ids, parents, src_row, rows_per_sample, row_ref);
  HIP_CHECK(hipGetLastError());
}

template <typename F>
void launch(mv_engine* e, const char* name, double flops, double bytes, F&& fn,
            double flops_dense = -1.0, double mfma_factor = 0.0) {
  if (!e->profiling) {
    fn();
    return;
  }
  int si = e->stat_index(name);
  PendingEvent pe{si, nullptr, nullptr};
  HIP_CHECK(hipEventCreate(&pe.a));
  HIP_CHECK(hipEventCreate(&pe.b));
  HIP_CHECK(hipEventRecord(pe.a, e->stream));
  fn();
  HIP_CHECK(hipEventRecord(pe.b, e->stream));
  e->stats[si].launches += 1;
  e->stats[si].flops += flops;
  e->stats[si].flops_dense += flops_dense >= 0 ? flops_dense : flops;
  e->stats[si].flops_mfma += mfma_factor * flops;
  e->stats[si].bytes += bytes;
  e->pending.push_back(pe);
}

void drain_events(mv_engine* e) {
  for (auto& pe : e->pending) {
    float ms = 0.f;
    HIP_CHECK(hipEventSynchronize(pe.b));
    HIP_CHECK(hipEventElapsedTime(&ms, pe.a, pe.b));
    e->stats[pe.stat].total_ms += ms;
    (void)hipEventDestroy(pe.a);
    (void)hipEventDestroy(pe.b);
  }
  e->pending.clear();
}


void build_param_table(mv_engine* e) {
  const mv_config& c = e->cfg;
  const int64_t C = c.hidden_size, D = c.scene_conv_dim, E = c.emb_size,
                k = c.convlstm_kernel, sk = c.scene_conv_kernel;
  int64_t cin = c.scene_class;
  char nm[256];
  if (e->no_scene()) {
    e->enc_emb_W = e->add_param("person_pred/grid_emb/W", {3, 3, 1, E});
    e->enc_emb_b = e->add_param("person_pred/grid_emb/b", {E});
  }
  for (int i = 0; i < c.num_scales && !e->no_scene(); ++i) {
    snprintf(nm, sizeof(nm), "person_pred/scene_conv%d/W", i + 1);
    e->scene_W.push_back(e->add_param(nm, {sk, sk, cin, D}));
    snprintf(nm, sizeof(nm), "person_pred/scene_conv%d/b", i + 1);
    e->scene_b.push_back(e->add_param(nm, {D}));
    cin = D;
  }
  for (int s = 0; s < c.num_scales; ++s) {
    ScaleState& S = e->sc[s];
    S.H = c.grid_h[s]; S.W = c.grid_w[s]; S.K = S.H * S.W;
    S.use = c.use_grid[s] != 0;
    if (!S.use) continue;
    auto cell = [&](ConvCell& cc, const char* fmt, int64_t Cx) {
      char base[200];
      snprintf(base, sizeof(base), fmt, s, s);
      cc.Cx = (int)Cx;
      cc.kernel = e->add_param(std::string("person_pred/") + base + "/kernel",
                               {k, k, Cx + C, 4 * C});
      cc.biases = e->add_param(std::string("person_pred/") + base + "/biases", {4 * C});
    };
    cell(S.enc_cls, "encoder_grid_class_%d/enc_grid_%d", e->no_scene() ? E : D);
    cell(S.enc_reg, "encoder_grid_reg_%d/enc_grid_regress_%d", 2);
    cell(S.dec_cls, "decoder_grid_class_%d/decoder_rnn/dec_grid_%d", E);
    snprintf(nm, sizeof(nm), "person_pred/decoder_grid_class_%d/decoder_rnn/grid_emb/W", s);
    S.emb_cls_W = e->add_param(nm, {3, 3, 1, E});
    snprintf(nm, sizeof(nm), "person_pred/decoder_grid_class_%d/decoder_rnn/grid_emb/b", s);
    S.emb_cls_b = e->add_param(nm, {E});
    snprintf(nm, sizeof(nm), "person_pred/hidden2grid_decoder_grid_class_%d/out_dec_grid/W", s);
    S.out_cls_W = e->add_param(nm, {3, 3, C, 1});
    if (c.use_single_decoder) {
      S.enc_reg.kernel->no_grad = S.enc_reg.biases->no_grad = true;
      if (!e->decode_reg_W)
        e->decode_reg_W = e->add_param("person_pred/decode_reg/out_dec_grid/W", {3, 3, C, 2});
      S.out_reg_W = e->decode_reg_W;
      continue;
    }
    cell(S.dec_reg, "decoder_grid_reg_%d/decoder_rnn/dec_grid_reg_%d", E);
    snprintf(nm, sizeof(nm), "person_pred/decoder_grid_reg_%d/decoder_rnn/grid_emb/W", s);
    S.emb_reg_W = e->add_param(nm, {3, 3, 2, E});
    snprintf(nm, sizeof(nm), "person_pred/decoder_grid_reg_%d/decoder_rnn/grid_emb/b", s);
    S.emb_reg_b = e->add_param(nm, {E});
    snprintf(nm, sizeof(nm), "person_pred/hidden2grid_decoder_grid_reg_%d/out_dec_grid/W", s);
    S.out_reg_W = e->add_param(nm, {3, 3, C, 2});
  }
}

std::vector<ConvCell*> active_cells(const mv_engine* e, ScaleState& S) {
  if (e->cfg.use_single_decoder) return {&S.enc_cls, &S.dec_cls};
  return {&S.enc_cls, &S.enc_reg, &S.dec_cls, &S.dec_reg};
}

void validate_config(const mv_config& c) {
  MV_REQUIRE(c.abi_version == MV_ABI_VERSION, "mv_config.abi_version %d != %d",
             c.abi_version, MV_ABI_VERSION);
  MV_REQUIRE(c.activation >= 0 && c.activation <= 2, "mv_config.activation %d (0 tanh, 1 relu, "
             "2 lrelu; reference code/pred_utils.py:86-94)", c.activation);
  MV_REQUIRE(c.batch_size > 0 && c.obs_len > 0 && c.max_pred_len > 0,
             "batch_size/obs_len/max_pred_len must be positive");
  MV_REQUIRE(c.num_scales >= 1 && c.num_scales <= MV_MAX_SCALES,
             "num_scales %d not in [1,%d]", c.num_scales, MV_MAX_SCALES);
  MV_REQUIRE(c.hidden_size == 128 || c.hidden_size == 256 || c.hidden_size == 512,
             "hidden_size %d unsupported (128, 256 or 512)", c.hidden_size);
  MV_REQUIRE(c.convlstm_kernel >= 1 && c.convlstm_kernel <= 9,
             "convlstm_kernel %d unsupported (1 .. 9)", c.convlstm_kernel);
  MV_REQUIRE(c.scene_conv_dim == 0 ||
             (c.scene_conv_dim > 0 && c.scene_conv_dim <= 128 &&
              mv::convlstm_cx_supported(c.scene_conv_dim)),
             "scene_conv_dim %d unsupported (0 = no scene encoder, or a multiple of 32 up to "
             "128)", c.scene_conv_dim);
  MV_REQUIRE(c.emb_size >= 32 && c.emb_size % 32 == 0 && c.emb_size <= 512 &&
             mv::convlstm_cx_supported(c.emb_size),
             "emb_size %d unsupported (a multiple of 32 up to 512)", c.emb_size);
  MV_REQUIRE(c.beam_size >= 1, "beam_size must be >= 1");
  MV_REQUIRE(!(c.class_feedback_dense && c.beam_size > 1), "class_feedback_dense: greedy only "
             "(grid_decoder_beam_search always feeds one-hot ids)");
  int hh = c.scene_h, ww = c.scene_w, used = 0;
  for (int s = 0; s < c.num_scales; ++s) {
    hh = (hh + 1) / 2; ww = (ww + 1) / 2;
    MV_REQUIRE(c.grid_h[s] == hh && c.grid_w[s] == ww,
               "scene_grids[%d] = %dx%d does not match the stride-2 conv chain "
               "(%dx%d); only scene_grid_strides 2,4,.. are supported",
               s, c.grid_h[s], c.grid_w[s], hh, ww);
    used += c.use_grid[s] != 0;
  }
  MV_REQUIRE(used >= 1, "no grid scale enabled");
  if (c.beam_size > 1)
    MV_REQUIRE(used == 1, "beam search: only one scale at a time "
               "(reference pred_models.py:262)");
}

void alloc_buffers(mv_engine* e) {
  const mv_config& c = e->cfg;
  const size_t N = c.batch_size, T = c.obs_len, Tp = c.max_pred_len,
               C = c.hidden_size, D = c.scene_conv_dim, B = c.beam_size;
  const size_t maxU = N * T;
  const bool scene = !e->no_scene();
  e->obs_scene.alloc(N * T);
  if (scene) e->scene_feat.alloc(maxU * c.scene_h * c.scene_w * c.scene_class);
  int hh = c.scene_h, ww = c.scene_w;
  for (int i = 0; i < c.num_scales; ++i) {
    hh = (hh + 1) / 2; ww = (ww + 1) / 2;
    e->conv_h.push_back(hh); e->conv_w.push_back(ww);
    if (scene) e->scene_conv[i].alloc(maxU * hh * ww * D);
  }
  const size_t xc = (size_t)std::max((int)D, c.emb_size);
  for (int s = 0; s < c.num_scales; ++s) {
    ScaleState& S = e->sc[s];
    if (!S.use) continue;
    const size_t K = S.K, R = N * B;
    S.scene_mean.alloc(N * K * std::max<size_t>(D, 1));
    if (!scene) HIP_CHECK(hipMemset(S.scene_mean.p, 0, N * K * sizeof(float)));
    S.labels.alloc(N * T);
    S.obs_reg.alloc(N * T * K * 2);
    for (int i = 0; i < 2; ++i) {
      S.cls_c[i].alloc(R * K * C); S.cls_h[i].alloc(R * K * C);
      S.reg_c[i].alloc(N * K * C); S.reg_h[i].alloc(N * K * C);
    }
    if (c.use_gnn) S.cls_hg.alloc(R * K * C);
    S.xbuf_cls.alloc(R * K * xc);
    S.xbuf_reg.alloc(N * K * xc);
    S.out_cls.alloc(N * Tp * K);
    S.out_reg.alloc(N * Tp * K * 2);
    S.ids.alloc(R);
    S.q_cls.alloc(R * K * 9); S.q_reg.alloc((c.use_single_decoder ? R : N) * K * 18);
    S.wq_cls.alloc(C * 32); S.wq_reg.alloc(C * 32);
    S.sx_cellyx.alloc(K);
    S.sx_dec_bias.alloc(9 * 4 * C); S.sx_dec_corr.alloc(9 * 25 * 4 * C);
    if (scene) S.sx_enc_corr.alloc(T * N * 9 * 4 * C);
    else { S.sx_enc_bias.alloc(9 * 4 * C); S.sx_enc_tab.alloc(9 * 25 * 4 * C); }
    if (B > 1) {
      e->bm_logits.alloc(Tp * R * K);
      e->bm_ids.alloc(Tp * R);
      e->bm_parents.alloc(Tp * R);
      e->bm_lp[0].alloc(R); e->bm_lp[1].alloc(R);
      e->bm_cand.alloc((size_t)R * K);
      e->bm_src_row.alloc(R);
      e->bm_ref.alloc(R);
      e->bm_trace.alloc(R * Tp);
      e->bm_out_logits.alloc(R * Tp * K);
      e->bm_out_ids.alloc(R * Tp);
      if (c.use_single_decoder) {
        e->bm_reg_steps.alloc(Tp * R * K * 2);
        e->bm_out_reg.alloc(R * Tp * K * 2);
      }
    }
  }
}

void ensure_packed(mv_engine* e, ConvCell& cc) {
  MV_REQUIRE(cc.kernel->set, "parameter %s not set", cc.kernel->name.c_str());
  MV_REQUIRE(cc.biases->set, "parameter %s not set", cc.biases->name.c_str());
  if (cc.wpack.p) return;
  if (e->cfg.convlstm_kernel != 3) return;
  const int C = e->cfg.hidden_size;
  std::vector<float> packed(mv::convlstm_wpack_elems(cc.Cx, C));
  mv::pack_convlstm_weights(cc.kernel->host.data(), cc.Cx, C, packed.data());
  cc.wpack.alloc(packed.size());
  HIP_CHECK(hipMemcpy(cc.wpack.p, packed.data(), packed.size() * sizeof(float),
                      hipMemcpyHostToDevice));
}

CellPacks packs_of(const mv_engine* e, const ConvCell& cc) {
  return cell_packs(e->compute_mode, e->cfg.activation, cc.Cx, e->cfg.hidden_size,
                    cc.wino_numerics_ok);
}

std::vector<float> kernel_h_rows(const float* kernel, int Cx, int C) {
  const int Cin = Cx + C, N4 = 4 * C;
  std::vector<float> wh((size_t)9 * C * N4);
  for (int t = 0; t < 9; ++t)
    memcpy(&wh[(size_t)t * C * N4], &kernel[((size_t)t * Cin + Cx) * N4],
           (size_t)C * N4 * sizeof(float));
  return wh;
}
std::vector<float> small_x_chunk(const float* kernel, int Cx, int C, float scale) {
  std::vector<float> packed(mv::convlstm_wpack_elems(Cx, C));
  mv::pack_convlstm_weights(kernel, Cx, C, packed.data());
  const int nch = mv::convlstm_xchunks(Cx) + 9 * (C / mv::kBK);
  std::vector<float> wx((size_t)(C / mv::kChBlock) * mv::kBN * mv::kBK);
  for (int cb = 0; cb < C / mv::kChBlock; ++cb)
    for (int i = 0; i < mv::kBN * mv::kBK; ++i)
      wx[(size_t)cb * mv::kBN * mv::kBK + i] =
          packed[((size_t)cb * nch + 0) * mv::kBN * mv::kBK + i] * scale;
  return wx;
}
template <typename T>
void upload(DevBuf<T>& dst, const std::vector<T>& src) {
  dst.alloc(src.size());
  HIP_CHECK(hipMemcpy(dst.p, src.data(), src.size() * sizeof(T), hipMemcpyHostToDevice));
}
void refresh_host_copy(ConvCell& cc) {
  if (!cc.host_stale) return;
  HIP_CHECK(hipMemcpy(cc.kernel->host.data(), cc.kernel->dev.p,
                      cc.kernel->elems() * sizeof(float), hipMemcpyDeviceToHost));
  cc.host_stale = false;
}

void ensure_packed16(mv_engine* e, ConvCell& cc) {
  if (cc.wp16.p) return;
  const int C = e->cfg.hidden_size;
  MV_REQUIRE(mv::f16x3_cx_supported(cc.Cx), "f16x3: Cx %d unsupported", cc.Cx);
  refresh_host_copy(cc);
  {
    float mx = 0.f;
    for (float v : cc.kernel->host) mx = std::max(mx, std::fabs(v));
    float reach = mx;
    if (cell_packs(1, e->cfg.activation, cc.Cx, C, true).wpw) {
      const size_t Cin = (size_t)cc.Cx + C, N4 = 4 * (size_t)C;
      const float* w = cc.kernel->host.data();
      for (size_t dxc = 0; dxc < 3 * Cin; ++dxc) {
        const size_t dx = dxc / Cin, ci = dxc - dx * Cin;
        const float* g0 = w + ((0 * 3 + dx) * Cin + ci) * N4;
        const float* g1 = w + ((1 * 3 + dx) * Cin + ci) * N4;
        const float* g2 = w + ((2 * 3 + dx) * Cin + ci) * N4;
        for (size_t n = 0; n < N4; ++n) {
          const float a = g0[n], b = g1[n], c2 = g2[n];
          const float t = std::max(std::max(std::fabs(a + b + c2), std::fabs(a - b + c2)) * 0.5f,
                                   std::max(std::fabs(a + 2.f * b + 4.f * c2),
                                            std::fabs(4.f * a + 2.f * b + c2)) * (1.f / 6.f));
          reach = std::max(reach, t);
        }
      }
    }
    MV_REQUIRE(reach * mv::kF16Scale < 60000.f, "f16x3: |%s| reaches %g (%g in the transformed "
               "kernel planes of the Winograd forms), outside the scaled fp16 range; use compute "
               "mode f32", cc.kernel->name.c_str(), mx, reach);
    std::vector<float> mag(cc.kernel->host.size());
    for (size_t i = 0; i < mag.size(); ++i) mag[i] = std::fabs(cc.kernel->host[i]);
    std::nth_element(mag.begin(), mag.begin() + mag.size() / 2, mag.end());
    const float med = mag[mag.size() / 2];
    const bool ok = mx <= kWinoOutlierRatio * med;
    if (!ok && cc.wino_numerics_ok)
      fprintf(stderr, "[multiverse_hip] f16x3: %s has max |w| %g at a median |w| of %g (> %g x): "
              "its gate convolution takes the direct 3x3 form instead of a Winograd form "
              "(roundoff of outlier weights would reach unrelated outputs)\n",
              cc.kernel->name.c_str(), mx, med, kWinoOutlierRatio);
    if (ok != cc.wino_numerics_ok) { cc.wpw.release(); cc.wpw3.release(); }
    cc.wino_numerics_ok = ok;
  }
  std::vector<_Float16> p16(mv::f16x3_wpack_elems(x_chunk16(cc.Cx), C));
  if (x_is_small(cc.Cx)) {
    mv::pack_f16x3_weights(kernel_h_rows(cc.kernel->host.data(), cc.Cx, C).data(), 0, C, p16.data());
    upload(cc.wx32, small_x_chunk(cc.kernel->host.data(), cc.Cx, C, 65536.0f));
  } else {
    mv::pack_f16x3_weights(cc.kernel->host.data(), cc.Cx, C, p16.data());
  }
  upload(cc.wp16, p16);
}

void pack_wino(hipStream_t stream, const float* w, int Cx, int C, DevBuf<_Float16>& dst) {
  const size_t halves = mv::wino_wpack_elems(x_chunk16(Cx), C);
  mv::wino_init_attributes();
  dst.alloc(halves);
  hipLaunchKernelGGL(mv::pack_wino_kernel, dim3(cdiv(halves / 2, 256)), dim3(256), 0, stream, w,
                     dst.p, Cx, x_chunk16(Cx), C, halves / 2);
}
void pack_wino3(hipStream_t stream, const float* w, int Cx, int C, DevBuf<_Float16>& dst) {
  const size_t halves = mv::wino3_wpack_elems(x_chunk16(Cx), C, mv::kW3Nrb);
  mv::wino3_init_attributes();
  dst.alloc(halves);
  hipLaunchKernelGGL(mv::pack_wino3_kernel, dim3(cdiv(halves / 2, 256)), dim3(256), 0, stream, w,
                     dst.p, Cx, x_chunk16(Cx), C, mv::kW3Nrb, halves / 2);
}
void pack_bf16t(hipStream_t stream, const float* w, int Cx, int C, DevBuf<_Float16>& dst) {
  const size_t halves = mv::bf16t_wpack_elems(x_chunk16(Cx), C, mv::kW3Nrb);
  dst.alloc(halves);
  hipLaunchKernelGGL(mv::pack_bf16t_kernel, dim3(cdiv(halves, 256)), dim3(256), 0, stream, w,
                     dst.p, Cx, x_chunk16(Cx), C, mv::kW3Nrb, halves);
}
void pack_tile_forms(mv_engine* e, ConvCell& cc) {
  const CellPacks p = packs_of(e, cc);
  const int C = e->cfg.hidden_size;
  if (e->compute_mode == 1) {
    if (p.wpw) pack_wino(e->stream, cc.kernel->dev.p, cc.Cx, C, cc.wpw); else cc.wpw.release();
    if (p.wpw3) pack_wino3(e->stream, cc.kernel->dev.p, cc.Cx, C, cc.wpw3); else cc.wpw3.release();
  } else if (e->compute_mode == 2) {
    if (p.wpbt) pack_bf16t(e->stream, cc.kernel->dev.p, cc.Cx, C, cc.wpbt); else cc.wpbt.release();
  }
}

void ensure_packed_bf16(mv_engine* e, ConvCell& cc) {
  if (cc.wpb.p) return;
  const int C = e->cfg.hidden_size;
  MV_REQUIRE(mv::f16x3_cx_supported(cc.Cx), "bf16: Cx %d unsupported", cc.Cx);
  refresh_host_copy(cc);
  const bool xf16 = bf16_x_passes(2, e->dyn_x(), x_is_small(cc.Cx)) == 3;
  std::vector<_Float16> pb(mv::bf16_wpack_elems(x_chunk16(cc.Cx), C, xf16));
  if (x_is_small(cc.Cx)) {
    mv::pack_bf16_weights(kernel_h_rows(cc.kernel->host.data(), cc.Cx, C).data(), 0, C, pb.data());
    upload(cc.wx32u, small_x_chunk(cc.kernel->host.data(), cc.Cx, C, 1.0f));
  } else {
    if (xf16) {
      const int Cin = cc.Cx + C, N4 = 4 * C;
      float mx = 0.f;
      for (int t = 0; t < 9; ++t)
        for (int ci = 0; ci < cc.Cx; ++ci)
          for (int n = 0; n < N4; ++n)
            mx = std::max(mx, std::fabs(cc.kernel->host[((size_t)t * Cin + ci) * N4 + n]));
      MV_REQUIRE(mx * mv::kF16Scale < 60000.f, "bf16 mode, unbounded activations: the x rows of "
                 "%s reach %g, outside the scaled fp16 range; use compute mode f32",
                 cc.kernel->name.c_str(), mx);
    }
    mv::pack_bf16_weights(cc.kernel->host.data(), cc.Cx, C, pb.data(), xf16);
  }
  upload(cc.wpb, pb);
  pack_tile_forms(e, cc);
}

int gnn_scene_dim(const mv_engine* e) {
  return (e->cfg.simaug_graph && e->cfg.beam_size == 1) ? 0 : e->cfg.scene_conv_dim;
}

bool sparse_x_on(const mv_engine* e, const ScaleState& S) {
  static const bool off = getenv("MV_SPARSE_X") && atoi(getenv("MV_SPARSE_X")) == 0;
  const mv_config& c = e->cfg;
  return !off && e->compute_mode != 0 && !e->train && S.use && S.H >= 3 && S.W >= 3 &&
         S.dec_cls.Cx == c.emb_size && c.emb_size % 16 == 0 && c.scene_conv_dim % 16 == 0 &&
         c.scene_conv_dim <= 64;
}

void ensure_params(mv_engine* e) {
  for (auto& p : e->params)
    MV_REQUIRE(p->set, "parameter %s not set (mv_set_param)", p->name.c_str());
  for (int s = 0; s < e->cfg.num_scales; ++s) {
    ScaleState& S = e->sc[s];
    if (!S.use) continue;
    for (ConvCell* cc : active_cells(e, S)) ensure_packed(e, *cc);
    if (e->compute_mode == 1)
      for (ConvCell* cc : active_cells(e, S)) ensure_packed16(e, *cc);
    if (e->compute_mode == 1)
      for (ConvCell* cc : active_cells(e, S))
        if (packs_of(e, *cc).wpw && !cc->wpw.p) pack_tile_forms(e, *cc);
    if (e->compute_mode == 2)
      for (ConvCell* cc : active_cells(e, S)) ensure_packed_bf16(e, *cc);
    if (!S.wq_valid) {
      const int C = e->cfg.hidden_size;
      hipLaunchKernelGGL(mv::pack_h2g_kernel, dim3(cdiv((size_t)C * 32, 256)), dim3(256), 0,
                         e->stream, S.out_cls_W->dev.p, S.wq_cls.p, C, 1);
      hipLaunchKernelGGL(mv::pack_h2g_kernel, dim3(cdiv((size_t)C * 32, 256)), dim3(256), 0,
                         e->stream, S.out_reg_W->dev.p, S.wq_reg.p, C, 2);
      S.wq_valid = true;
    }
    if (!S.sx_valid && sparse_x_on(e, S)) {
      const int C = e->cfg.hidden_size;
      hipLaunchKernelGGL(mv::cell_yx_kernel, dim3(cdiv((size_t)S.K, 256)), dim3(256), 0,
                         e->stream, S.sx_cellyx.p, S.H, S.W);
      hipLaunchKernelGGL(mv::sx_decoder_tables_kernel,
                         dim3(cdiv((size_t)(9 + 9 * 25) * 4 * C, 256)), dim3(256), 0, e->stream,
                         S.dec_cls.kernel->dev.p, S.dec_cls.biases->dev.p, S.emb_cls_W->dev.p,
                         S.emb_cls_b->dev.p, S.dec_cls.Cx, C, S.sx_dec_bias.p, S.sx_dec_corr.p,
                         e->cfg.activation);
      if (e->no_scene())
        hipLaunchKernelGGL(mv::sx_decoder_tables_kernel,
                           dim3(cdiv((size_t)(9 + 9 * 25) * 4 * C, 256)), dim3(256), 0,
                           e->stream, S.enc_cls.kernel->dev.p, S.enc_cls.biases->dev.p,
                           e->enc_emb_W->dev.p, e->enc_emb_b->dev.p, S.enc_cls.Cx, C,
                           S.sx_enc_bias.p, S.sx_enc_tab.p, e->cfg.activation);
      S.sx_valid = true;
    }
  }
}

}
```

### multiverse_amd/csrc/engine_state.h

```cpp
#pragma once

struct mv_train_holder;

namespace {

thread_local std::string g_create_error;



struct HipError { std::string msg; };

#define HIP_CHECK(expr)                                                       \
  do {                                                                        \
    hipError_t _e = (expr);                                                   \
    if (_e != hipSuccess) {                                                   \
      char _b[512];                                                           \
      snprintf(_b, sizeof(_b), "%s failed: %s (%s:%d)", #expr,                \
               hipGetErrorString(_e), __FILE__, __LINE__);                    \
      throw HipError{_b};                                                     \
    }                                                                         \
  } while (0)

#define MV_REQUIRE(cond, ...)                                                 \
  do {                                                                        \
    if (!(cond)) {                                                            \
      char _b[512];                                                           \
      snprintf(_b, sizeof(_b), __VA_ARGS__);                                  \
      throw HipError{_b};                                                     \
    }                                                                         \
  } while (0)

template <typename T>
struct DevBuf {
  T* p = nullptr;
  T* base = nullptr;
  size_t n = 0;
  void alloc(size_t count, size_t pad = 0) {
    if (count <= n && p) return;
    release();
    HIP_CHECK(hipMalloc(reinterpret_cast<void**>(&base), (count + 2 * pad) * sizeof(T)));
    if (pad) HIP_CHECK(hipMemset(base, 0, (count + 2 * pad) * sizeof(T)));
    p = base + pad;
    n = count;
  }
  void release() {
    if (base) (void)hipFree(base);
    p = nullptr; base = nullptr; n = 0;
  }
  ~DevBuf() { release(); }
  DevBuf() = default;
  DevBuf(const DevBuf&) = delete;
  DevBuf& operator=(const DevBuf&) = delete;
};

struct Param {
  std::string name;
  std::vector<int64_t> shape;
  std::vector<float> host;
  DevBuf<float> dev;
  bool set = false;
  bool no_grad = false;
  size_t elems() const {
    size_t e = 1;
    for (auto d : shape) e *= (size_t)d;
    return e;
  }
};

struct ConvCell {
  Param* kernel = nullptr;
  Param* biases = nullptr;
  DevBuf<float> wpack;
  DevBuf<_Float16> wp16;
  DevBuf<float> wx32;
  DevBuf<_Float16> wpb;
  DevBuf<float> wx32u;
  DevBuf<_Float16> wpw;
  DevBuf<_Float16> wpw3;
  DevBuf<_Float16> wpbt;
  bool host_stale = false;
  bool wino_numerics_ok = true;
  int Cx = 0;
};
constexpr float kWinoOutlierRatio = 4096.f;

struct KernelStat {
  std::string name;
  int64_t launches = 0;
  double total_ms = 0, flops = 0, bytes = 0, flops_dense = 0;
  double flops_mfma = 0;
};

struct PendingEvent {
  int stat;
  hipEvent_t a, b;
};

struct ScaleState {
  int H = 0, W = 0, K = 0;
  bool use = false;
  ConvCell enc_cls, enc_reg, dec_cls, dec_reg;
  Param *emb_cls_W = nullptr, *emb_cls_b = nullptr, *emb_reg_W = nullptr,
        *emb_reg_b = nullptr, *out_cls_W = nullptr, *out_reg_W = nullptr;
  DevBuf<float> scene_mean;
  DevBuf<int32_t> labels;
  DevBuf<float> obs_reg;
  DevBuf<double> centers;
  DevBuf<float> cls_c[2], cls_h[2], cls_hg;
  DevBuf<float> reg_c[2], reg_h[2];
  DevBuf<float> xbuf_cls, xbuf_reg;
  DevBuf<float> out_cls;
  DevBuf<float> out_reg;
  DevBuf<int32_t> ids;
  DevBuf<float> q_cls, q_reg;
  DevBuf<float> wq_cls, wq_reg;
  bool wq_valid = false;
  DevBuf<uint32_t> sx_cellyx;
  DevBuf<float> sx_dec_bias, sx_dec_corr;
  DevBuf<float> sx_enc_corr;
  DevBuf<float> sx_enc_bias, sx_enc_tab;
  bool sx_valid = false;
};

}

struct mv_engine {
  mv_config cfg{};
  int device = 0;
  hipStream_t stream = nullptr;
  std::string err;
  std::vector<std::unique_ptr<Param>> params;
  Param* decode_reg_W = nullptr;
  std::map<std::string, Param*> by_name;
  std::vector<Param*> scene_W, scene_b;
  Param *enc_emb_W = nullptr, *enc_emb_b = nullptr;
  bool no_scene() const { return cfg.scene_conv_dim == 0; }
  ScaleState sc[MV_MAX_SCALES];
  DevBuf<int32_t> obs_scene;
  DevBuf<float> scene_feat;
  DevBuf<uint8_t> scene_u8;
  DevBuf<double> xy_dev;
  DevBuf<float> scene_conv[MV_MAX_SCALES];
  std::vector<int> conv_h, conv_w;
  int num_frames = 0;
  int pred_len = 0;
  bool inputs_ready = false;
  DevBuf<float> bm_logits;
  DevBuf<int32_t> bm_ids, bm_parents;
  DevBuf<float> bm_lp[2];
  DevBuf<float> bm_cand;
  DevBuf<int32_t> bm_src_row;
  DevBuf<int32_t> bm_ref;
  DevBuf<int32_t> bm_trace;
  DevBuf<float> bm_out_logits;
  DevBuf<float> bm_reg_steps;
  DevBuf<float> bm_out_reg;
  DevBuf<int32_t> bm_out_ids;
  int last_forward = 0;
  DevBuf<double> mf_traj;
  DevBuf<float> mf_occ;
  int compute_mode = 0;
  DevBuf<_Float16> px16[mv::kMaxGroup], ph16[mv::kMaxGroup];
  DevBuf<_Float16> pv3x[mv::kMaxGroup], pv3h[mv::kMaxGroup];
  DevBuf<int32_t> xexp[mv::kMaxGroup];
  std::set<const float*> xbufs;
  bool dyn_x() const { return compute_mode != 0 && cfg.activation != 0; }
  struct PlaneBuf { _Float16* p; size_t n; bool valid; };
  std::map<const float*, PlaneBuf> planes;
  std::vector<std::unique_ptr<DevBuf<_Float16>>> plane_store;
  _Float16* plane_out(const float* dst, size_t* stride) {
    if (compute_mode == 0) return nullptr;
    if (dyn_x() && xbufs.count(dst)) return nullptr;
    auto it = planes.find(dst);
    if (it == planes.end()) return nullptr;
    it->second.valid = true;
    *stride = compute_mode == 2 ? 0 : it->second.n;
    return it->second.p;
  }
  void plane_invalidate(const float* dst) {
    auto it = planes.find(dst);
    if (it != planes.end()) it->second.valid = false;
  }
  bool graph_mode = false;
  std::map<std::tuple<int, int, int>, hipGraphExec_t> graphs;
  void drop_graphs() {
    for (auto& kv : graphs) (void)hipGraphExecDestroy(kv.second);
    graphs.clear();
  }
  struct PipeSlot {
    void* pin = nullptr;
    char* dev = nullptr;
    size_t in_bytes = 0, out_bytes = 0;
    hipEvent_t h2d = nullptr, done = nullptr, d2h = nullptr;
    int num_frames = 0, pred_len = 0;
    bool busy = false;
  };
  std::vector<PipeSlot> pipe;
  hipStream_t copy_stream = nullptr;
  hipStream_t fetch_stream = nullptr;
  size_t pipe_head = 0, pipe_tail = 0;
  mv::Comm* comm = nullptr;
  mv_train_holder* train = nullptr;
  bool train_packs_valid = false;
  bool profiling = false;
  std::vector<KernelStat> stats;
  std::vector<PendingEvent> pending;

  Param* add_param(const std::string& name, std::vector<int64_t> shape) {
    params.emplace_back(new Param());
    Param* p = params.back().get();
    p->name = name;
    p->shape = std::move(shape);
    by_name[name] = p;
    return p;
  }
  int stat_index(const char* name) {
    for (size_t i = 0; i < stats.size(); ++i)
      if (stats[i].name == name) return (int)i;
    stats.push_back(KernelStat{name});
    return (int)stats.size() - 1;
  }
};
```

Measured before the change: 4261 trajectories/sec.

## Run class and regression ConvLSTM chains on two concurrent streams

Splits the greedy forward into two independent chains, class and regression. Each chain issues its gate groups on its own HIP stream, with fork and join events around the forward. Separate scratch-slot ranges keep the f16 plane buffers from conflicting, and both chains share one joint forward plan. The aim is to overlap small, latency-bound per-timestep kernels of the two chains so the GPU stays busier at batch 64. In exchange it adds stream and event management and scratch aliasing concerns, and it is disabled under graph capture and profiling.

Measured after the change: 4329 trajectories/sec, median of 6. 1.02x the previous value.

```diff
diff --git a/multiverse_amd/csrc/engine.hip b/multiverse_amd/csrc/engine.hip
--- a/multiverse_amd/csrc/engine.hip
+++ b/multiverse_amd/csrc/engine.hip
@@ -90,6 +90,8 @@
     e->cfg = *cfg;
     e->device = device;
     HIP_CHECK(hipStreamCreate(&e->stream));
+    e->issue = e->stream;
+    create_chain_streams(e);
     build_param_table(e);
     alloc_buffers(e);
     if (cfg->beam_size > 1) {
@@ -99,7 +101,15 @@
       ensure_beam_step_lds(device, ((size_t)2 * cfg->beam_size * K + 512) * sizeof(float));
     }
   });
-  if (rc != 0) { delete e; return rc; }
+  if (rc != 0) {
+    if (e) {
+      if (e->fork_ev) (void)hipEventDestroy(e->fork_ev);
+      if (e->join_ev) (void)hipEventDestroy(e->join_ev);
+      if (e->stream_b) (void)hipStreamDestroy(e->stream_b);
+    }
+    delete e;
+    return rc;
+  }
   *out = e;
   return 0;
 }
@@ -108,6 +118,7 @@
   if (!h) return 0;
   (void)hipSetDevice(h->device);
   if (h->stream) (void)hipStreamSynchronize(h->stream);
+  if (h->stream_b) (void)hipStreamSynchronize(h->stream_b);
   if (h->copy_stream) (void)hipStreamSynchronize(h->copy_stream);
   if (h->fetch_stream) (void)hipStreamSynchronize(h->fetch_stream);
   pipeline_destroy(h);
@@ -121,6 +132,9 @@
     delete h->comm;
   }
   delete h->train;
+  if (h->fork_ev) (void)hipEventDestroy(h->fork_ev);
+  if (h->join_ev) (void)hipEventDestroy(h->join_ev);
+  if (h->stream_b) (void)hipStreamDestroy(h->stream_b);
   if (h->stream) (void)hipStreamDestroy(h->stream);
   delete h;
   return 0;
diff --git a/multiverse_amd/csrc/engine_forward.h b/multiverse_amd/csrc/engine_forward.h
--- a/multiverse_amd/csrc/engine_forward.h
+++ b/multiverse_amd/csrc/engine_forward.h
@@ -71,6 +71,7 @@
   for (size_t i = 0; i < probs.size(); ++i) {
     const ConvLstmArgs& a = probs[i];
     mv::ConvLstm16Args& q = p16[i];
+    const size_t sl = (size_t)e->slot0 + i;
     MV_REQUIRE(a.H * a.W >= 32, "f16x3 / bf16 compute modes need grids of at least 32 cells "
                "(%d x %d); use compute mode f32", a.H, a.W);
     MV_REQUIRE((double)a.rows * a.H * a.W * a.C * 4.0 < 4294967296.0,
@@ -110,13 +111,13 @@
         q.x16 = pb->p; q.x_plane_stride = (int64_t)pb->n;
       } else {
         const size_t pst = ncell * a.Cx + mv::kPlaneSlack + mv::kPlanePad;
-        MV_REQUIRE(e->px16[i].n >= 2 * pst, "internal: f16x3 x plane scratch");
-        _Float16* p0 = e->px16[i].p + mv::kPlanePad;
+        MV_REQUIRE(e->px16[sl].n >= 2 * pst, "internal: f16x3 x plane scratch");
+        _Float16* p0 = e->px16[sl].p + mv::kPlanePad;
         q.x16 = p0; q.x_plane_stride = (int64_t)pst;
         if (e->dyn_x()) {
-          MV_REQUIRE(e->xexp[i].p, "internal: x exponent scratch");
-          q.x_exp = e->xexp[i].p + 64;
-          dyn_splits.push_back(DynItem{a.x, p0, p0 + pst, (int)ncell, a.Cx, e->xexp[i].p});
+          MV_REQUIRE(e->xexp[sl].p, "internal: x exponent scratch");
+          q.x_exp = e->xexp[sl].p + 64;
+          dyn_splits.push_back(DynItem{a.x, p0, p0 + pst, (int)ncell, a.Cx, e->xexp[sl].p});
         } else {
           splits.push_back(SplitItem{a.x, p0, bf16 ? (_Float16*)nullptr : p0 + pst, (int)ncell, a.Cx});
         }
@@ -129,8 +130,8 @@
         q.h16 = pb->p; q.h_plane_stride = (int64_t)pb->n;
       } else {
         const size_t pst = ncell * a.C + mv::kPlaneSlack + mv::kPlanePad;
-        MV_REQUIRE(e->ph16[i].n >= 2 * pst, "internal: f16x3 h plane scratch");
-        _Float16* p0 = e->ph16[i].p + mv::kPlanePad;
+        MV_REQUIRE(e->ph16[sl].n >= 2 * pst, "internal: f16x3 h plane scratch");
+        _Float16* p0 = e->ph16[sl].p + mv::kPlanePad;
         q.h16 = p0; q.h_plane_stride = (int64_t)pst;
         splits.push_back(SplitItem{a.h, p0, bf16 ? (_Float16*)nullptr : p0 + pst, (int)ncell, a.C});
       }
@@ -138,12 +139,12 @@
   }
   for (const DynItem& it : dyn_splits) {
     launch(e, "split_planes", 0, 12.0 * (double)it.cells * it.C, [&] {
-      HIP_CHECK(hipMemsetAsync(it.bits, 0, 64 * sizeof(int32_t), e->stream));
-      hipLaunchKernelGGL(mv::absmax_bits_kernel, dim3(256), dim3(256), 0, e->stream, it.in,
+      HIP_CHECK(hipMemsetAsync(it.bits, 0, 64 * sizeof(int32_t), e->issue));
+      hipLaunchKernelGGL(mv::absmax_bits_kernel, dim3(256), dim3(256), 0, e->issue, it.in,
                          (size_t)it.cells * it.C, it.bits);
       hipLaunchKernelGGL(mv::split_planes_dyn_kernel,
                          dim3(mv::split_planes_blocks((size_t)it.cells, it.C)), dim3(256), 0,
-                         e->stream, it.in, it.p0, it.p1, it.cells, it.C, it.bits, it.bits + 64);
+                         e->issue, it.in, it.p0, it.p1, it.cells, it.C, it.bits, it.bits + 64);
     });
   }
   for (size_t s0 = 0; s0 < splits.size(); s0 += mv::kSplitGroup) {
@@ -159,7 +160,7 @@
       sbytes += (bf16 ? 6.0 : 8.0) * (double)it.cells * it.C;
     }
     launch(e, "split_planes", 0, sbytes, [&] {
-      hipLaunchKernelGGL(mv::split_planes_group_kernel, dim3(nb), dim3(256), 0, e->stream, g);
+      hipLaunchKernelGGL(mv::split_planes_group_kernel, dim3(nb), dim3(256), 0, e->issue, g);
     });
   }
 }
@@ -191,64 +192,102 @@
   else mv::launch_convlstm_bf16t_steps(pw, n, pl.halo, pl.map_mode, stream);
 }
 
-void run_conv_group_f16x3(mv_engine* e, const std::vector<ConvLstmArgs>& probs,
-                          double flops, double bytes, double dense) {
+struct GatePrep {
+  std::vector<ConvCell*> cells;
+  std::vector<mv::ConvLstm16Args> p16;
+  int slot0 = 0;
+  double flops = 0, bytes = 0, dense = 0;
+  int n() const { return (int)p16.size(); }
+};
+
+void gate_group_cost(const std::vector<ConvLstmArgs>& probs, double& flops, double& bytes,
+                     double& dense) {
+  flops = bytes = dense = 0;
+  for (const auto& a : probs) {
+    const double M = (double)a.rows * a.H * a.W;
+    dense += 2.0 * M * 9.0 * (a.Cx + a.C) * 4.0 * a.C;
+    const double cx = a.sx_corr ? 0.0 : (double)a.Cx;
+    flops += 2.0 * M * 9.0 * (cx + (a.zero_state ? 0 : a.C)) * 4.0 * a.C;
+    bytes += M * (cx + (a.zero_state ? 2.0 : 4.0) * a.C) * 4.0;
+  }
+}
+
+GatePrep prepare_gate_group(mv_engine* e, const std::vector<ConvLstmArgs>& probs) {
+  GatePrep g;
   const int n = (int)probs.size();
-  MV_REQUIRE(n <= mv::kMaxGroup, "internal: gate group of %d problems", n);
-  std::vector<ConvCell*> cells(n);
-  for (int i = 0; i < n; ++i) cells[i] = cell_of_pack(e, probs[i].wpack);
-  std::vector<mv::ConvLstm16Args> p16(n);
-  prepare_gate_operands(e, probs, cells, p16);
+  MV_REQUIRE(e->slot0 + n <= mv::kMaxGroup, "internal: gate group of %d problems from slot %d",
+             n, e->slot0);
+  g.slot0 = e->slot0;
+  g.cells.resize(n);
+  for (int i = 0; i < n; ++i) g.cells[i] = cell_of_pack(e, probs[i].wpack);
+  g.p16.resize(n);
+  prepare_gate_operands(e, probs, g.cells, g.p16);
+  gate_group_cost(probs, g.flops, g.bytes, g.dense);
+  return g;
+}
+
+ForwardPlan plan_gate_groups(mv_engine* e, const GatePrep* const* groups, int ngroups) {
   ForwardProblem fp[mv::kMaxGroup];
-  for (int i = 0; i < n; ++i) fp[i] = ForwardProblem{&p16[i], cells[i], e->pv3x[i].n, e->pv3h[i].n};
-  const ForwardPlan pl = plan_forward_group(e->compute_mode, fp, n);
+  int n = 0;
+  for (int g = 0; g < ngroups; ++g)
+    for (int i = 0; i < groups[g]->n(); ++i) {
+      MV_REQUIRE(n < mv::kMaxGroup, "internal: more than %d gate problems in a step", mv::kMaxGroup);
+      const int sl = groups[g]->slot0 + i;
+      fp[n++] = ForwardProblem{&groups[g]->p16[i], groups[g]->cells[i], e->pv3x[sl].n, e->pv3h[sl].n};
+    }
+  return plan_forward_group(e->compute_mode, fp, n);
+}
+
+void issue_gate_group(mv_engine* e, const GatePrep& g, const ForwardPlan& pl) {
+  const int n = g.n();
   const _Float16* packs[mv::kMaxGroup] = {};
   const float* w_hwio[mv::kMaxGroup] = {};
   _Float16 *v3x[mv::kMaxGroup] = {}, *v3h[mv::kMaxGroup] = {};
   std::vector<mv::Wn3TransformItem> tr3;
   double tr3_bytes = 0;
   for (int i = 0; i < n; ++i) {
-    const mv::ConvLstm16Args& q = p16[i];
+    const mv::ConvLstm16Args& q = g.p16[i];
     const ConvLstmArgs& a = q.f;
-    w_hwio[i] = cells[i]->kernel->dev.p;
-    packs[i] = pl.form == GateForm::Wino2 ? cells[i]->wpw.p
-             : pl.form == GateForm::Wino3 ? cells[i]->wpw3.p
-             : pl.form == GateForm::Bf16T ? cells[i]->wpbt.p : nullptr;
+    const int sl = g.slot0 + i;
+    w_hwio[i] = g.cells[i]->kernel->dev.p;
+    packs[i] = pl.form == GateForm::Wino2 ? g.cells[i]->wpw.p
+             : pl.form == GateForm::Wino3 ? g.cells[i]->wpw3.p
+             : pl.form == GateForm::Bf16T ? g.cells[i]->wpbt.p : nullptr;
     if (pl.form != GateForm::Wino3) continue;
     if (!a.zero_state) {
-      v3h[i] = e->pv3h[i].p;
+      v3h[i] = e->pv3h[sl].p;
       tr3_bytes += queue_wino3_transform(tr3, {q.h16, q.h_plane_stride, v3h[i], a.src_row_h,
                                                a.rows, a.H, a.W, a.C});
     }
     if (has_dense_x(a)) {
-      v3x[i] = e->pv3x[i].p;
+      v3x[i] = e->pv3x[sl].p;
       tr3_bytes += queue_wino3_transform(tr3, {q.x16, q.x_plane_stride, v3x[i], nullptr,
                                                a.rows, a.H, a.W, a.Cx});
     }
   }
   if (!tr3.empty())
     launch(e, "wino3_transform", 0, tr3_bytes, [&] {
-      mv::launch_wino3_transforms(tr3.data(), (int)tr3.size(), e->stream);
+      mv::launch_wino3_transforms(tr3.data(), (int)tr3.size(), e->issue);
     });
-  launch(e, "convlstm_step", flops, bytes, [&] {
-    launch_gate_group(pl, p16.data(), packs, w_hwio, v3x, v3h, n, e->stream);
-  }, dense, pl.mfma_factor);
+  launch(e, "convlstm_step", g.flops, g.bytes, [&] {
+    launch_gate_group(pl, g.p16.data(), packs, w_hwio, v3x, v3h, n, e->issue);
+  }, g.dense, pl.mfma_factor);
+}
+
+void run_conv_group_f16x3(mv_engine* e, const std::vector<ConvLstmArgs>& probs) {
+  const GatePrep g = prepare_gate_group(e, probs);
+  const GatePrep* gp = &g;
+  issue_gate_group(e, g, plan_gate_groups(e, &gp, 1));
 }
 
 void run_conv_group(mv_engine* e, const std::vector<ConvLstmArgs>& probs) {
   if (probs.empty()) return;
+  if (e->compute_mode != 0) {
+    run_conv_group_f16x3(e, probs);
+    return;
+  }
   double flops = 0, bytes = 0, dense = 0;
-  for (const auto& a : probs) {
-    const double M = (double)a.rows * a.H * a.W;
-    dense += 2.0 * M * 9.0 * (a.Cx + a.C) * 4.0 * a.C;
-    const double cx = a.sx_corr ? 0.0 : (double)a.Cx;
-    flops += 2.0 * M * 9.0 * (cx + (a.zero_state ? 0 : a.C)) * 4.0 * a.C;
-    bytes += M * (cx + (a.zero_state ? 2.0 : 4.0) * a.C) * 4.0;
-  }
-  if (e->compute_mode != 0) {
-    run_conv_group_f16x3(e, probs, flops, bytes, dense);
-    return;
-  }
+  gate_group_cost(probs, flops, bytes, dense);
   if (e->cfg.convlstm_kernel != 3) {
     const double kk = (double)e->cfg.convlstm_kernel * e->cfg.convlstm_kernel / 9.0;
     launch(e, "convlstm_step", flops * kk, bytes, [&] {
@@ -257,14 +296,32 @@
         ga.f = a;
         ga.w = cell_of_bias(e, a.bias)->kernel->dev.p;
         ga.ksize = e->cfg.convlstm_kernel;
-        mv::launch_convlstm_generic_step(ga, e->stream);
+        mv::launch_convlstm_generic_step(ga, e->issue);
       }
     }, dense * kk, 0.0);
     return;
   }
   launch(e, "convlstm_step", flops, bytes, [&] {
-    mv::launch_convlstm_steps(probs.data(), (int)probs.size(), e->stream);
+    mv::launch_convlstm_steps(probs.data(), (int)probs.size(), e->issue);
   }, dense, 1.0);
+}
+
+void run_conv_pairs(mv_engine* e, const std::vector<ConvLstmArgs>& a,
+                    const std::vector<ConvLstmArgs>& b) {
+  if (e->compute_mode == 0 || a.empty() || b.empty()) {
+    { IssueOn on(e, 0); run_conv_group(e, a); }
+    { IssueOn on(e, 1); run_conv_group(e, b); }
+    return;
+  }
+  MV_REQUIRE(a.size() <= 2 && b.size() <= 2, "internal: chain pairs of %zu / %zu problems",
+             a.size(), b.size());
+  GatePrep ga, gb;
+  { IssueOn on(e, 0); ga = prepare_gate_group(e, a); }
+  { IssueOn on(e, 1); gb = prepare_gate_group(e, b); }
+  const GatePrep* both[2] = {&gb, &ga};
+  const ForwardPlan pl = plan_gate_groups(e, both, 2);
+  { IssueOn on(e, 0); issue_gate_group(e, ga, pl); }
+  { IssueOn on(e, 1); issue_gate_group(e, gb, pl); }
 }
 
 void run_scene(mv_engine* e) {
@@ -285,13 +342,13 @@
       launch(e, "scene_proj1x1_mfma", 2.0 * M * Ci * Co,
              4.0 * (total + (double)M * Ci), [&] {
         hipLaunchKernelGGL(mv::scene_proj1x1_mfma_kernel, dim3(cdiv(M, 128)), dim3(256), 0,
-                           e->stream, in, w, b, out, U, Hi, Wi, Ci, Ho, Wo, Co, c.activation);
+                           e->issue, in, w, b, out, U, Hi, Wi, Ci, Ho, Wo, Co, c.activation);
       });
     } else {
     launch(e, "scene_conv_s2_tanh", 2.0 * total * k * k * Ci,
            4.0 * (total + (double)U * Hi * Wi * Ci), [&] {
       hipLaunchKernelGGL(mv::scene_conv_s2_tanh_kernel, dim3(cdiv(total, 256)),
-                         dim3(256), 0, e->stream, in, w, b, out, U, Hi, Wi, Ci,
+                         dim3(256), 0, e->issue, in, w, b, out, U, Hi, Wi, Ci,
                          Ho, Wo, Co, k, pad_h / 2, pad_w / 2, c.activation);
     });
     }
@@ -304,7 +361,7 @@
     launch(e, "scene_mean", (double)total * c.obs_len,
            4.0 * total * (c.obs_len + 1), [&] {
       hipLaunchKernelGGL(mv::scene_mean_kernel, dim3(cdiv(total, 256)), dim3(256),
-                         0, e->stream, e->scene_conv[s].p, e->obs_scene.p,
+                         0, e->issue, e->scene_conv[s].p, e->obs_scene.p,
                          S.scene_mean.p, c.batch_size, c.obs_len, S.K,
                          c.scene_conv_dim);
     });
@@ -322,14 +379,17 @@
   return on;
 }
 
-void run_encoders(mv_engine* e, Cursors& cur) {
+enum : int { kChainCls = 1, kChainReg = 2, kChainAll = 3 };
+
+void encoder_step_problems(mv_engine* e, Cursors& cur, int t, int chains,
+                           std::vector<ConvLstmArgs>& probs) {
   const mv_config& c = e->cfg;
   const int N = c.batch_size, T = c.obs_len, D = c.scene_conv_dim;
-  for (int t = 0; t < T; ++t) {
-    std::vector<ConvLstmArgs> probs;
-    for (int s = 0; s < c.num_scales; ++s) {
+  for (int s = 0; s < c.num_scales; ++s) {
+    {
       ScaleState& S = e->sc[s];
       if (!S.use) continue;
+      if (chains & kChainCls) {
       const size_t total = (size_t)N * S.K * D;
       const bool sparse = sparse_x_on(e, S);
       const size_t nc = (size_t)N * 9 * 4 * c.hidden_size;
@@ -341,7 +401,7 @@
             size_t pst = 0;
             _Float16* p16 = e->plane_out(S.xbuf_cls.p, &pst);
             hipLaunchKernelGGL(mv::enc_grid_emb_onehot_kernel, dim3(cdiv(tx, 256)), dim3(256),
-                               0, e->stream, S.labels.p, T, t, 1, e->enc_emb_W->dev.p,
+                               0, e->issue, S.labels.p, T, t, 1, e->enc_emb_W->dev.p,
                                e->enc_emb_b->dev.p, S.xbuf_cls.p, N, S.H, S.W, E, p16, pst,
                                c.activation);
           });
@@ -352,7 +412,7 @@
             hipLaunchKernelGGL(mv::sx_encoder_corr_kernel,
                                dim3(cdiv((size_t)4 * c.hidden_size, 256), 9,
                                     cdiv((size_t)N, mv::kSxRows) * T),
-                               dim3(256), 0, e->stream, S.enc_cls.kernel->dev.p,
+                               dim3(256), 0, e->issue, S.enc_cls.kernel->dev.p,
                                e->scene_conv[s].p, e->obs_scene.p, S.labels.p, N, T, -1, S.K, D,
                                c.hidden_size, S.sx_enc_corr.p);
           });
@@ -361,13 +421,12 @@
         size_t pst = 0;
         _Float16* p16 = e->plane_out(S.xbuf_cls.p, &pst);
         hipLaunchKernelGGL(mv::enc_class_input_kernel, dim3(cdiv(total, 256)),
-                           dim3(256), 0, e->stream, e->scene_conv[s].p,
+                           dim3(256), 0, e->issue, e->scene_conv[s].p,
                            e->obs_scene.p, S.labels.p, S.xbuf_cls.p, N, T, t, S.K, D, p16,
                            pst);
       });
       }
-      const size_t row = (size_t)S.K * 2;
-      const int cc = cur.cls[s], cr = cur.reg[s];
+      const int cc = cur.cls[s];
       probs.push_back(conv_problem(e, S.enc_cls, S.xbuf_cls.p, S.cls_h[cc].p,
                                    S.cls_c[cc].p, nullptr, nullptr, S.cls_h[cc ^ 1].p,
                                    S.cls_c[cc ^ 1].p, N, S.H, S.W, t == 0, 0,
@@ -382,15 +441,34 @@
         set_sparse_x(e, S, probs.back(), false, S.labels.p + t, T, 1);
         probs.back().sx_corr = S.sx_enc_corr.p + (size_t)t * nc;
       }
+      cur.cls[s] ^= 1;
+      }
+      if (!(chains & kChainReg)) continue;
+      const size_t row = (size_t)S.K * 2;
+      const int cr = cur.reg[s];
       if (!c.use_single_decoder)
         probs.push_back(conv_problem(e, S.enc_reg, S.obs_reg.p + (size_t)t * row,
                                      S.reg_h[cr].p, S.reg_c[cr].p, nullptr, nullptr,
                                      S.reg_h[cr ^ 1].p, S.reg_c[cr ^ 1].p, N, S.H, S.W,
                                      t == 0, (size_t)T * row));
       if (!c.use_single_decoder) probs.back().skip_h32 = 1;
-      cur.cls[s] ^= 1; cur.reg[s] ^= 1;
-    }
-    run_conv_group(e, probs);
+      cur.reg[s] ^= 1;
+    }
+  }
+}
+
+void run_encoders(mv_engine* e, Cursors& cur, bool pairs) {
+  for (int t = 0; t < e->cfg.obs_len; ++t) {
+    if (!pairs) {
+      std::vector<ConvLstmArgs> probs;
+      encoder_step_problems(e, cur, t, kChainAll, probs);
+      run_conv_group(e, probs);
+      continue;
+    }
+    std::vector<ConvLstmArgs> pa, pb;
+    { IssueOn on(e, 0); encoder_step_problems(e, cur, t, kChainCls, pa); }
+    { IssueOn on(e, 1); encoder_step_problems(e, cur, t, kChainReg, pb); }
+    run_conv_pairs(e, pa, pb);
   }
 }
 
@@ -448,9 +526,9 @@
     launch(e, "gnn_attend", flops, bytes, [&] {
       if (tiled && ver >= 3) {
         hipLaunchKernelGGL(mv::gnn_attend_v3_kernel, dim3(nblocks), dim3(mv::kGnn3Threads), 0,
-                           e->stream, grp, c.hidden_size, gnn_scene_dim(e));
+                           e->issue, grp, c.hidden_size, gnn_scene_dim(e));
       } else if (tiled) {
-        hipLaunchKernelGGL(mv::gnn_attend_v2_kernel, dim3(nblocks), dim3(mv::kGnnThreads), 0, e->stream,
+        hipLaunchKernelGGL(mv::gnn_attend_v2_kernel, dim3(nblocks), dim3(mv::kGnnThreads), 0, e->issue,
                            grp, c.hidden_size, gnn_scene_dim(e));
       } else {
         const size_t cells = (size_t)A.rows * A.S->K;
@@ -458,11 +536,11 @@
         _Float16* p16 = e->plane_out(A.out, &pst);
         if (c.hidden_size <= 256)
           hipLaunchKernelGGL(mv::gnn_attend_kernel<1>, dim3(cdiv(cells, 4)), dim3(256), 0,
-                             e->stream, A.h, A.S->scene_mean.p, A.src_row, A.out, A.rows,
+                             e->issue, A.h, A.S->scene_mean.p, A.src_row, A.out, A.rows,
                              A.S->H, A.S->W, c.hidden_size, gnn_scene_dim(e), A.sm_div, p16, pst);
         else
           hipLaunchKernelGGL(mv::gnn_attend_kernel<2>, dim3(cdiv(cells, 4)), dim3(256), 0,
-                             e->stream, A.h, A.S->scene_mean.p, A.src_row, A.out, A.rows,
+                             e->issue, A.h, A.S->scene_mean.p, A.src_row, A.out, A.rows,
                              A.S->H, A.S->W, c.hidden_size, gnn_scene_dim(e), A.sm_div, p16, pst);
       }
     });
@@ -482,7 +560,7 @@
   const int C = e->cfg.hidden_size;
   launch(e, "hidden2grid", cells * 2.0 * 9 * C * P, 4.0 * cells * (C + P), [&] {
     hipLaunchKernelGGL(mv::hidden2grid_kernel<P>, dim3(cdiv(cells, 4)), dim3(256),
-                       0, e->stream, h, w, out, out_row_stride, rows, S.H, S.W, C);
+                       0, e->issue, h, w, out, out_row_stride, rows, S.H, S.W, C);
   });
 }
 
@@ -500,11 +578,11 @@
     _Float16* p16 = e->plane_out(out, &pst);
     if (tail_v2() && E % 8 == 0)
       hipLaunchKernelGGL(mv::grid_emb_onehot8_kernel, dim3(cdiv(total / 8, 256)), dim3(256), 0,
-                         e->stream, ids, stride, ids_div, S.emb_cls_W->dev.p,
+                         e->issue, ids, stride, ids_div, S.emb_cls_W->dev.p,
                          S.emb_cls_b->dev.p, out, rows, S.H, S.W, E, p16, pst, e->cfg.activation);
     else
       hipLaunchKernelGGL(mv::grid_emb_onehot_kernel, dim3(cdiv(total, 256)),
-                         dim3(256), 0, e->stream, ids, stride, ids_div, S.emb_cls_W->dev.p,
+                         dim3(256), 0, e->issue, ids, stride, ids_div, S.emb_cls_W->dev.p,
                          S.emb_cls_b->dev.p, out, rows, S.H, S.W, E, p16, pst, e->cfg.activation);
   });
 }
@@ -518,7 +596,7 @@
     size_t pst = 0;
     _Float16* p16 = e->plane_out(out, &pst);
     hipLaunchKernelGGL(mv::grid_emb_dense_kernel, dim3(cdiv(total, 256)), dim3(256),
-                       0, e->stream, x, row_stride, W->dev.p, b->dev.p, out, rows, S.H, S.W,
+                       0, e->issue, x, row_stride, W->dev.p, b->dev.p, out, rows, S.H, S.W,
                        P, E, p16, pst, e->cfg.activation);
   });
 }
@@ -555,6 +633,7 @@
   int reg_rows = 0;
   int32_t* cls_ids_out = nullptr; float* cls_x_out = nullptr; float* reg_x_out = nullptr;
   bool cls_embed = true;
+  bool do_cls = true, do_reg = true;
 };
 
 void run_tail(mv_engine* e, const std::vector<TailPlan>& plans) {
@@ -569,10 +648,17 @@
                "decode tail: K %d / emb_size %d", S.K, E);
     const int reg_rows = pl.reg_rows ? pl.reg_rows : N;
     const size_t cc = (size_t)pl.cls_rows * S.K, cr = (size_t)reg_rows * S.K;
-    qp.push_back(mv::H2gQProblem{pl.cls_h, S.wq_cls.p, S.q_cls.p, (int32_t)cc, 1});
-    qp.push_back(mv::H2gQProblem{pl.reg_h, S.wq_reg.p, S.q_reg.p, (int32_t)cr, 2});
-    qbytes += 4.0 * (cc * (C + 9.0) + cr * (C + 18.0));
-    qflops += 2.0 * 9 * C * (cc + 2.0 * cr);
+    if (pl.do_cls) {
+      qp.push_back(mv::H2gQProblem{pl.cls_h, S.wq_cls.p, S.q_cls.p, (int32_t)cc, 1});
+      qbytes += 4.0 * cc * (C + 9.0);
+      qflops += 2.0 * 9 * C * cc;
+    }
+    if (pl.do_reg) {
+      qp.push_back(mv::H2gQProblem{pl.reg_h, S.wq_reg.p, S.q_reg.p, (int32_t)cr, 2});
+      qbytes += 4.0 * cr * (C + 18.0);
+      qflops += 2.0 * 9 * C * 2.0 * cr;
+    }
+    if (pl.do_cls) {
     mv::TailProblem a{};
     a.q = S.q_cls.p; a.out = pl.cls_out; a.out_row_stride = pl.cls_stride;
     a.rows = pl.cls_rows; a.H = S.H; a.W = S.W; a.P = 1; a.E = E; a.onehot = 1;
@@ -595,6 +681,8 @@
       }
     }
     tp.push_back(a);
+    }
+    if (!pl.do_reg) continue;
     mv::TailProblem b{};
     b.q = S.q_reg.p; b.out = pl.reg_out; b.out_row_stride = pl.reg_stride;
     b.rows = reg_rows; b.H = S.H; b.W = S.W; b.P = 2; b.E = E; b.onehot = 0;
@@ -615,59 +703,65 @@
     tp.push_back(b);
   }
   MV_REQUIRE(qp.size() <= (size_t)mv::kTailMax, "decode tail: too many chains");
+  if (qp.empty()) return;
   launch(e, "hidden2grid", qflops, qbytes, [&] {
-    mv::launch_h2g_q(qp.data(), (int)qp.size(), C, e->stream);
+    mv::launch_h2g_q(qp.data(), (int)qp.size(), C, e->issue);
   });
   launch(e, "decode_tail", 0, tbytes, [&] {
-    mv::launch_decode_tail(tp.data(), (int)tp.size(), e->stream);
+    mv::launch_decode_tail(tp.data(), (int)tp.size(), e->issue);
   });
 }
 
-void run_decoders_greedy(mv_engine* e, Cursors& cur, int Tp) {
+void run_decoders_greedy(mv_engine* e, Cursors& cur, int Tp, bool pairs) {
   const mv_config& c = e->cfg;
   const int N = c.batch_size, T = c.obs_len;
   const bool v2 = tail_v2();
+  MV_REQUIRE(!pairs || (v2 && !c.use_single_decoder), "internal: chain pairs need the grouped "
+             "decoder tail and a regression decoder");
   for (int t = 0; t < Tp; ++t) {
-    std::vector<ConvLstmArgs> probs;
-    if (c.use_gnn) {
-      std::vector<GnnJob> jobs;
-      for (int s = 0; s < c.num_scales; ++s)
-        if (e->sc[s].use)
-          jobs.push_back(GnnJob{&e->sc[s], e->sc[s].cls_h[cur.cls[s]].p, nullptr,
-                                e->sc[s].cls_hg.p, N, 1});
-      run_gnn_jobs(e, jobs);
-    }
-    for (int s = 0; s < c.num_scales; ++s) {
-      ScaleState& S = e->sc[s];
-      if (!S.use) continue;
-      const int cc = cur.cls[s];
-      const float* hin = c.use_gnn ? S.cls_hg.p : S.cls_h[cc].p;
-      const bool sparse = sparse_x_on(e, S) && (t == 0 || !c.class_feedback_dense);
-      if (sparse)
-        ;
-      else if (t == 0)
-        run_emb_onehot(e, S, S.labels.p + (T - 1), T, S.xbuf_cls.p, N);
-      else if (c.class_feedback_dense)
-        run_emb_dense(e, S, S.out_cls.p + (size_t)(t - 1) * S.K, (size_t)Tp * S.K,
-                      S.xbuf_cls.p, N, S.emb_cls_W, S.emb_cls_b, 1);
-      else if (!v2)
-        run_emb_onehot(e, S, S.ids.p, 1, S.xbuf_cls.p, N);
-      probs.push_back(conv_problem(e, S.dec_cls, S.xbuf_cls.p, hin, S.cls_c[cc].p,
-                                   nullptr, nullptr, S.cls_h[cc ^ 1].p,
-                                   S.cls_c[cc ^ 1].p, N, S.H, S.W, false, 0,
-                                   !c.use_gnn));
-      if (sparse) {
-        if (t == 0) set_sparse_x(e, S, probs.back(), true, S.labels.p + (T - 1), T, 1);
-        else set_sparse_x(e, S, probs.back(), true, S.ids.p, 1, 1);
-      }
-      cur.cls[s] ^= 1;
-      if (!c.use_single_decoder) probs.push_back(reg_decoder_problem(e, s, cur, t, Tp, !v2));
-    }
-    std::stable_sort(probs.begin(), probs.end(), [](const ConvLstmArgs& a, const ConvLstmArgs& b) {
-      return (a.sx_corr == nullptr) > (b.sx_corr == nullptr);
-    });
-    run_conv_group(e, probs);
-    if (v2) {
+    auto step_problems = [&](int chains, std::vector<ConvLstmArgs>& probs) {
+      if ((chains & kChainCls) && c.use_gnn) {
+        std::vector<GnnJob> jobs;
+        for (int s = 0; s < c.num_scales; ++s)
+          if (e->sc[s].use)
+            jobs.push_back(GnnJob{&e->sc[s], e->sc[s].cls_h[cur.cls[s]].p, nullptr,
+                                  e->sc[s].cls_hg.p, N, 1});
+        run_gnn_jobs(e, jobs);
+      }
+      for (int s = 0; s < c.num_scales; ++s) {
+        ScaleState& S = e->sc[s];
+        if (!S.use) continue;
+        if (chains & kChainCls) {
+          const int cc = cur.cls[s];
+          const float* hin = c.use_gnn ? S.cls_hg.p : S.cls_h[cc].p;
+          const bool sparse = sparse_x_on(e, S) && (t == 0 || !c.class_feedback_dense);
+          if (sparse)
+            ;
+          else if (t == 0)
+            run_emb_onehot(e, S, S.labels.p + (T - 1), T, S.xbuf_cls.p, N);
+          else if (c.class_feedback_dense)
+            run_emb_dense(e, S, S.out_cls.p + (size_t)(t - 1) * S.K, (size_t)Tp * S.K,
+                          S.xbuf_cls.p, N, S.emb_cls_W, S.emb_cls_b, 1);
+          else if (!v2)
+            run_emb_onehot(e, S, S.ids.p, 1, S.xbuf_cls.p, N);
+          probs.push_back(conv_problem(e, S.dec_cls, S.xbuf_cls.p, hin, S.cls_c[cc].p,
+                                       nullptr, nullptr, S.cls_h[cc ^ 1].p,
+                                       S.cls_c[cc ^ 1].p, N, S.H, S.W, false, 0,
+                                       !c.use_gnn));
+          if (sparse) {
+            if (t == 0) set_sparse_x(e, S, probs.back(), true, S.labels.p + (T - 1), T, 1);
+            else set_sparse_x(e, S, probs.back(), true, S.ids.p, 1, 1);
+          }
+          cur.cls[s] ^= 1;
+        }
+        if ((chains & kChainReg) && !c.use_single_decoder)
+          probs.push_back(reg_decoder_problem(e, s, cur, t, Tp, !v2));
+      }
+      std::stable_sort(probs.begin(), probs.end(), [](const ConvLstmArgs& a, const ConvLstmArgs& b) {
+        return (a.sx_corr == nullptr) > (b.sx_corr == nullptr);
+      });
+    };
+    auto step_tail = [&](int chains) {
       std::vector<TailPlan> plans;
       for (int s = 0; s < c.num_scales; ++s) {
         ScaleState& S = e->sc[s];
@@ -684,9 +778,26 @@
           pl.reg_h = pl.cls_h;
           pl.reg_next = false;
         }
+        pl.do_cls = (chains & kChainCls) != 0;
+        pl.do_reg = (chains & kChainReg) != 0;
         plans.push_back(pl);
       }
       run_tail(e, plans);
+    };
+    if (pairs) {
+      std::vector<ConvLstmArgs> pa, pb;
+      { IssueOn on(e, 0); step_problems(kChainCls, pa); }
+      { IssueOn on(e, 1); step_problems(kChainReg, pb); }
+      run_conv_pairs(e, pa, pb);
+      { IssueOn on(e, 0); step_tail(kChainCls); }
+      { IssueOn on(e, 1); step_tail(kChainReg); }
+      continue;
+    }
+    std::vector<ConvLstmArgs> probs;
+    step_problems(kChainAll, probs);
+    run_conv_group(e, probs);
+    if (v2) {
+      step_tail(kChainAll);
       continue;
     }
     for (int s = 0; s < c.num_scales; ++s) {
@@ -697,7 +808,7 @@
       run_hidden2grid<1>(e, S, S.cls_h[cur.cls[s]].p, S.out_cls_W->dev.p, logits, orow, N);
       if (t + 1 < Tp && !c.class_feedback_dense) {
         launch(e, "argmax_rows", 0, 4.0 * N * S.K, [&] {
-          hipLaunchKernelGGL(mv::argmax_rows_kernel, dim3(N), dim3(64), 0, e->stream,
+          hipLaunchKernelGGL(mv::argmax_rows_kernel, dim3(N), dim3(64), 0, e->issue,
                              logits, orow, S.ids.p, N, S.K);
         });
       }
@@ -771,14 +882,14 @@
     const size_t row4 = (size_t)K * C / 4, total4 = (size_t)R * row4;
     launch(e, "beam_tile_state", 0, 8.0 * total4 * 16, [&] {
       hipLaunchKernelGGL(tile_rows_kernel, dim3(cdiv(total4, 256)), dim3(256), 0,
-                         e->stream, S.cls_h[cc].p, S.cls_h[cc ^ 1].p, row4, B, total4);
+                         e->issue, S.cls_h[cc].p, S.cls_h[cc ^ 1].p, row4, B, total4);
       hipLaunchKernelGGL(tile_rows_kernel, dim3(cdiv(total4, 256)), dim3(256), 0,
-                         e->stream, S.cls_c[cc].p, S.cls_c[cc ^ 1].p, row4, B, total4);
+                         e->issue, S.cls_c[cc].p, S.cls_c[cc ^ 1].p, row4, B, total4);
     });
     e->plane_invalidate(S.cls_h[cc ^ 1].p);
     cur.cls[s] ^= 1;
   }
-  HIP_CHECK(hipMemsetAsync(e->bm_lp[0].p, 0, (size_t)R * sizeof(float), e->stream));
+  HIP_CHECK(hipMemsetAsync(e->bm_lp[0].p, 0, (size_t)R * sizeof(float), e->issue));
   int lpi = 0;
   const int32_t* src = nullptr;
   const bool sparse = sparse_x_on(e, S);
@@ -835,17 +946,17 @@
       if (one_per_sample) {
         const size_t total = (size_t)R * K;
         hipLaunchKernelGGL(tile_beam0_kernel, dim3(cdiv(total, 256)), dim3(256), 0,
-                           e->stream, logits, K, B, total);
+                           e->issue, logits, K, B, total);
         if (single)
           hipLaunchKernelGGL(tile_beam0_kernel, dim3(cdiv(total * 2, 256)), dim3(256), 0,
-                             e->stream, regstep, K * 2, B, total * 2);
+                             e->issue, regstep, K * 2, B, total * 2);
       }
       int32_t* ids = e->bm_ids.p + (size_t)(time - 1) * R;
       int32_t* parents = e->bm_parents.p + (size_t)(time - 1) * R;
       if (dedupe)
-        HIP_CHECK(hipMemsetAsync(e->bm_ref.p, 0, (size_t)R * sizeof(int32_t), e->stream));
+        HIP_CHECK(hipMemsetAsync(e->bm_ref.p, 0, (size_t)R * sizeof(int32_t), e->issue));
       launch(e, "beam_step", 0, 4.0 * R * K, [&] {
-        launch_beam_step(e->stream, logits, e->bm_lp[lpi].p, e->bm_cand.p, N, B, K, time,
+        launch_beam_step(e->issue, logits, e->bm_lp[lpi].p, e->bm_cand.p, N, B, K, time,
                          c.diverse_beam, logf(c.diverse_gamma), c.fix_num_timestep,
                          e->bm_lp[lpi ^ 1].p, ids, parents, e->bm_src_row.p,
                          one_per_sample ? 1 : B, dedupe ? e->bm_ref.p : nullptr);
@@ -874,35 +985,47 @@
     }
   }
   hipLaunchKernelGGL(beam_backtrace_kernel, dim3(cdiv(R, 256)), dim3(256), 0,
-                     e->stream, e->bm_ids.p, e->bm_parents.p, e->bm_out_ids.p,
+                     e->issue, e->bm_ids.p, e->bm_parents.p, e->bm_out_ids.p,
                      e->bm_trace.p, N, B, Tp);
   const size_t total = (size_t)R * Tp * K;
   hipLaunchKernelGGL(beam_gather_logits_kernel, dim3(cdiv(total, 256)), dim3(256), 0,
-                     e->stream, e->bm_logits.p, e->bm_trace.p, e->bm_out_logits.p,
+                     e->issue, e->bm_logits.p, e->bm_trace.p, e->bm_out_logits.p,
                      N, B, Tp, K);
   if (c.use_single_decoder) {
     const size_t tot2 = (size_t)R * Tp * K * 2;
     hipLaunchKernelGGL(beam_gather_logits_kernel, dim3(cdiv(tot2, 256)), dim3(256), 0,
-                       e->stream, e->bm_reg_steps.p, e->bm_trace.p, e->bm_out_reg.p,
+                       e->issue, e->bm_reg_steps.p, e->bm_trace.p, e->bm_out_reg.p,
                        N, B, Tp, K * 2);
   }
   if (lpi != 0)
     HIP_CHECK(hipMemcpyAsync(e->bm_lp[0].p, e->bm_lp[1].p, (size_t)R * sizeof(float),
-                             hipMemcpyDeviceToDevice, e->stream));
-}
-
-void enqueue_forward(mv_engine* e, bool beam) {
+                             hipMemcpyDeviceToDevice, e->issue));
+}
+
+constexpr int kChainPairMaxBatch = 64;
+
+void enqueue_forward(mv_engine* e, bool beam, bool capturing = false) {
   const mv_config& c = e->cfg;
   const int Tp = e->pred_len;
+  const bool pairs = !beam && e->stream_b && !e->profiling && !capturing && c.beam_size == 1 &&
+                     !c.use_single_decoder && tail_v2() && c.batch_size <= kChainPairMaxBatch;
+  Cursors cur;
+  if (pairs) {
+    ChainFork fork(e);
+    if (!e->no_scene()) { IssueOn on(e, 0); run_scene(e); }
+    run_encoders(e, cur, true);
+    run_decoders_greedy(e, cur, Tp, true);
+    HIP_CHECK(hipGetLastError());
+    return;
+  }
   if (!e->no_scene()) run_scene(e);
-  Cursors cur;
-  run_encoders(e, cur);
+  run_encoders(e, cur, false);
   if (beam) {
     int s = 0;
     for (int i = 0; i < c.num_scales; ++i) if (e->sc[i].use) s = i;
     run_decoders_beam(e, s, cur, Tp);
   } else {
-    run_decoders_greedy(e, cur, Tp);
+    run_decoders_greedy(e, cur, Tp, false);
   }
   HIP_CHECK(hipGetLastError());
 }
@@ -923,7 +1046,7 @@
     hipGraph_t g = nullptr;
     HIP_CHECK(hipStreamBeginCapture(e->stream, hipStreamCaptureModeThreadLocal));
     try {
-      enqueue_forward(e, beam);
+      enqueue_forward(e, beam, true);
     } catch (...) {
       (void)hipStreamEndCapture(e->stream, &g);
       if (g) (void)hipGraphDestroy(g);
diff --git a/multiverse_amd/csrc/engine_setup.h b/multiverse_amd/csrc/engine_setup.h
--- a/multiverse_amd/csrc/engine_setup.h
+++ b/multiverse_amd/csrc/engine_setup.h
@@ -50,6 +50,58 @@
   HIP_CHECK(hipGetLastError());
 }
 
+static int chain_streams() {
+  static const int n = (getenv("MV_CHAIN_STREAMS") && atoi(getenv("MV_CHAIN_STREAMS")) == 1) ? 1 : 2;
+  return n;
+}
+static bool chain_priority() {
+  static const bool on = getenv("MV_CHAIN_PRIORITY") && atoi(getenv("MV_CHAIN_PRIORITY")) == 1;
+  return on;
+}
+
+void create_chain_streams(mv_engine* e) {
+  if (chain_streams() != 2) return;
+  if (chain_priority()) {
+    int least = 0, greatest = 0;
+    HIP_CHECK(hipDeviceGetStreamPriorityRange(&least, &greatest));
+    HIP_CHECK(hipStreamCreateWithPriority(&e->stream_b, hipStreamDefault, least));
+  } else {
+    HIP_CHECK(hipStreamCreate(&e->stream_b));
+  }
+  HIP_CHECK(hipEventCreateWithFlags(&e->fork_ev, hipEventDisableTiming));
+  HIP_CHECK(hipEventCreateWithFlags(&e->join_ev, hipEventDisableTiming));
+}
+
+struct IssueOn {
+  mv_engine* e;
+  hipStream_t prev;
+  int prev_slot0;
+  IssueOn(mv_engine* e_, int pair) : e(e_), prev(e_->issue), prev_slot0(e_->slot0) {
+    e->issue = pair ? e->stream_b : e->stream;
+    e->slot0 = pair ? 2 : 0;
+  }
+  ~IssueOn() { e->issue = prev; e->slot0 = prev_slot0; }
+  IssueOn(const IssueOn&) = delete;
+  IssueOn& operator=(const IssueOn&) = delete;
+};
+
+struct ChainFork {
+  mv_engine* e;
+  explicit ChainFork(mv_engine* e_) : e(e_) {
+    HIP_CHECK(hipEventRecord(e->fork_ev, e->stream));
+    HIP_CHECK(hipStreamWaitEvent(e->stream_b, e->fork_ev, 0));
+  }
+  ~ChainFork() {
+    e->issue = e->stream;
+    e->slot0 = 0;
+    if (hipEventRecord(e->join_ev, e->stream_b) != hipSuccess ||
+        hipStreamWaitEvent(e->stream, e->join_ev, 0) != hipSuccess)
+      (void)hipStreamSynchronize(e->stream_b);
+  }
+  ChainFork(const ChainFork&) = delete;
+  ChainFork& operator=(const ChainFork&) = delete;
+};
+
 template <typename F>
 void launch(mv_engine* e, const char* name, double flops, double bytes, F&& fn,
             double flops_dense = -1.0, double mfma_factor = 0.0) {
@@ -61,9 +113,9 @@
   PendingEvent pe{si, nullptr, nullptr};
   HIP_CHECK(hipEventCreate(&pe.a));
   HIP_CHECK(hipEventCreate(&pe.b));
-  HIP_CHECK(hipEventRecord(pe.a, e->stream));
+  HIP_CHECK(hipEventRecord(pe.a, e->issue));
   fn();
-  HIP_CHECK(hipEventRecord(pe.b, e->stream));
+  HIP_CHECK(hipEventRecord(pe.b, e->issue));
   e->stats[si].launches += 1;
   e->stats[si].flops += flops;
   e->stats[si].flops_dense += flops_dense >= 0 ? flops_dense : flops;
diff --git a/multiverse_amd/csrc/engine_state.h b/multiverse_amd/csrc/engine_state.h
--- a/multiverse_amd/csrc/engine_state.h
+++ b/multiverse_amd/csrc/engine_state.h
@@ -128,6 +128,10 @@
   mv_config cfg{};
   int device = 0;
   hipStream_t stream = nullptr;
+  hipStream_t stream_b = nullptr;
+  hipEvent_t fork_ev = nullptr, join_ev = nullptr;
+  hipStream_t issue = nullptr;
+  int slot0 = 0;
   std::string err;
   std::vector<std::unique_ptr<Param>> params;
   Param* decode_reg_W = nullptr;
```
